# pranoyr/attention-models

Hardware: AMD Instinct MI355X
Metric: ViTVQGAN 256px train-step images/sec (higher is better)
Workload: dtype f32; 1 GPU; BASELINE.json configs[2]: ViTVQGAN dim=256 patch=8 img=256 depth=6+6 h=8 d=64 mlp=2048 (SwiGLU), codebook 8192x32; GAN train step (D phase + G phase, gradient penalty, per_loss_weight=0), Adam, clip 1.0; global_batch=32, batch_per_gpu=32, parallelism=dp1

## Files before the change

attention-models_amd/amk/dense.py:

```python
import ctypes

import torch

from . import lib as _lib
from .lib import EPI_BIAS, EPI_RESID, EPI_SWIGLU, EPI_SWIGLU_BWD, GEMM_NN, GEMM_NT, GEMM_TN, GemmDesc


def _p(t):
    return ctypes.c_void_p(t.data_ptr()) if t is not None else ctypes.c_void_p(0)


def _stream():
    return ctypes.c_void_p(torch.cuda.current_stream().cuda_stream)


def _mat(t, what):
    if t is None:
        return None
    if not t.is_cuda:
        raise RuntimeError("amk ops run only on MI355X (HIP) tensors; got a CPU tensor. There is no CPU fallback.")
    if t.dtype != torch.float32:
        raise RuntimeError(f"amk kernels compute in fp32; got {t.dtype} for {what}")
    if t.dim() != 2:
        raise RuntimeError(f"{what} must be a matrix, got shape {tuple(t.shape)}")
    if t.stride(1) != 1 or t.stride(0) % 4 or t.data_ptr() % 16:
        t = t.contiguous()
    return t


def _vec(t, n, what):
    if t is None:
        return None
    if not t.is_cuda or t.dtype != torch.float32:
        raise RuntimeError(f"{what}: an fp32 HIP tensor is required")
    t = t.contiguous()
    if t.numel() != n:
        raise RuntimeError(f"{what}: {t.numel()} elements, expected {n}")
    return t


def supported(*dims):
    return all(d > 0 and d % 4 == 0 for d in dims)


def _run(d, ws=None):
    L = _lib.load()
    rc = L.amk_gemm_f32(ctypes.byref(d), _p(ws), ws.numel() * 4 if ws is not None else 0, _stream())
    _lib.check(rc, "amk_gemm_f32")


def _set_ln(d, ln, M, K):
    if ln is None:
        return ()
    mean, rstd, gamma, beta = ln
    keep = (_vec(mean, M, "ln mean"), _vec(rstd, M, "ln rstd"), _vec(gamma, K, "ln gamma"), _vec(beta, K, "ln beta"))
    d.ln_mean, d.ln_rstd, d.ln_gamma, d.ln_beta = (_p(t) for t in keep)
    return keep


def row_stats(x2, eps=1e-5):
    x2 = _mat(x2, "x")
    M, D = x2.shape
    if x2.stride(0) != D:
        x2 = x2.contiguous()
    mean = torch.empty((M,), device=x2.device, dtype=torch.float32)
    rstd = torch.empty_like(mean)
    _lib.check(_lib.load().amk_row_stats(_p(x2), M, D, float(eps), _p(mean), _p(rstd), _stream()), "amk_row_stats")
    return mean, rstd


def gemm_nt(a, w, bias=None, *, w2=None, bias2=None, resid=None, ln=None, out=None):
    a, w, w2, resid = _mat(a, "a"), _mat(w, "w"), _mat(w2, "w2"), _mat(resid, "resid")
    M, K = a.shape
    N1 = w.shape[0]
    N2 = w2.shape[0] if w2 is not None else 0
    if w.shape[1] != K or (w2 is not None and w2.shape[1] != K):
        raise RuntimeError(f"gemm_nt: a {tuple(a.shape)} against w {tuple(w.shape)}")
    c = out if out is not None else torch.empty((M, N1), device=a.device, dtype=torch.float32)
    c2 = torch.empty((M, N2), device=a.device, dtype=torch.float32) if w2 is not None else None
    d = GemmDesc(op=GEMM_NT, epilogue=EPI_RESID if resid is not None else EPI_BIAS, m=M, n=N1 + N2, k=K,
                 split=N1 if w2 is not None else 0)
    bias, bias2 = _vec(bias, N1, "bias"), _vec(bias2, N2, "bias2")
    d.a, d.lda, d.w, d.ldw, d.c, d.ldc, d.bias = _p(a), a.stride(0), _p(w), w.stride(0), _p(c), c.stride(0), _p(bias)
    if w2 is not None:
        d.w2, d.ldw2, d.c2, d.ldc2, d.bias2 = _p(w2), w2.stride(0), _p(c2), c2.stride(0), _p(bias2)
    if resid is not None:
        if resid.shape != (M, N1):
            raise RuntimeError(f"gemm_nt: resid {tuple(resid.shape)} against output {(M, N1)}")
        d.resid, d.ldr = _p(resid), resid.stride(0)
    keep = _set_ln(d, ln, M, K)
    _run(d)
    return (c, c2) if w2 is not None else c


def gemm_nt_swiglu(a, w12, b12=None, *, ln=None, keep_ab=True):
    a, w12 = _mat(a, "a"), _mat(w12, "w12")
    M, K = a.shape
    H = w12.shape[0] // 2
    if w12.shape[1] != K or w12.shape[0] != 2 * H:
        raise RuntimeError(f"gemm_nt_swiglu: a {tuple(a.shape)} against w12 {tuple(w12.shape)}")
    gate = torch.empty((M, H), device=a.device, dtype=torch.float32)
    ab = torch.empty((M, 2 * H), device=a.device, dtype=torch.float32) if keep_ab else None
    d = GemmDesc(op=GEMM_NT, epilogue=EPI_SWIGLU, m=M, n=H, k=K)
    b12 = _vec(b12, 2 * H, "b12")
    d.a, d.lda, d.w, d.ldw, d.bias = _p(a), a.stride(0), _p(w12), w12.stride(0), _p(b12)
    d.gate, d.ldg = _p(gate), H
    d.c, d.ldc = _p(ab), 2 * H
    keep = _set_ln(d, ln, M, K)
    _run(d)
    return gate, ab


def gemm_nn(a, w, *, a2=None, w2=None, swiglu_ab=None):
    a, w, a2, w2, swiglu_ab = _mat(a, "a"), _mat(w, "w"), _mat(a2, "a2"), _mat(w2, "w2"), _mat(swiglu_ab, "ab")
    M, K1 = a.shape
    N = w.shape[1]
    K2 = a2.shape[1] if a2 is not None else 0
    if w.shape[0] != K1 or (a2 is not None and (w2 is None or w2.shape != (K2, N) or a2.shape[0] != M)):
        raise RuntimeError(f"gemm_nn: a {tuple(a.shape)} against w {tuple(w.shape)}")
    width = 2 * N if swiglu_ab is not None else N
    c = torch.empty((M, width), device=a.device, dtype=torch.float32)
    d = GemmDesc(op=GEMM_NN, epilogue=EPI_SWIGLU_BWD if swiglu_ab is not None else EPI_BIAS, m=M, n=N, k=K1 + K2,
                 split=K1 if a2 is not None else 0)
    d.a, d.lda, d.w, d.ldw, d.c, d.ldc = _p(a), a.stride(0), _p(w), w.stride(0), _p(c), width
    if a2 is not None:
        d.a2, d.lda2, d.w2, d.ldw2 = _p(a2), a2.stride(0), _p(w2), w2.stride(0)
    if swiglu_ab is not None:
        if swiglu_ab.shape != (M, 2 * N):
            raise RuntimeError(f"gemm_nn: (a | b) {tuple(swiglu_ab.shape)} against dGate {(M, N)}")
        d.ab, d.ldab = _p(swiglu_ab), swiglu_ab.stride(0)
    _run(d)
    return c


def _out(t, shape, what):
    if t is None:
        return None
    if (not t.is_cuda or t.dtype != torch.float32 or tuple(t.shape) != tuple(shape) or not t.is_contiguous()
            or t.data_ptr() % 16):
        raise RuntimeError(f"{what}: an fp32 contiguous 16-byte aligned HIP tensor of shape {tuple(shape)} is required")
    return t


def gemm_tn(y, x, *, y2=None, ln=None, want_bias=False, out=None, out2=None, bias_out=None):
    y, x, y2 = _mat(y, "y"), _mat(x, "x"), _mat(y2, "y2")
    M, N1 = y.shape
    K = x.shape[1]
    N2 = y2.shape[1] if y2 is not None else 0
    if x.shape[0] != M or (y2 is not None and y2.shape[0] != M):
        raise RuntimeError(f"gemm_tn: y {tuple(y.shape)} against x {tuple(x.shape)}")
    dw = _out(out, (N1, K), "gemm_tn out")
    if dw is None:
        dw = torch.empty((N1, K), device=y.device, dtype=torch.float32)
    dw2 = None
    if y2 is not None:
        dw2 = _out(out2, (N2, K), "gemm_tn out2")
        if dw2 is None:
            dw2 = torch.empty((N2, K), device=y.device, dtype=torch.float32)
    db = None
    if want_bias:
        db = _out(bias_out, (N1 + N2,), "gemm_tn bias_out")
        if db is None:
            db = torch.empty((N1 + N2,), device=y.device, dtype=torch.float32)
    d = GemmDesc(op=GEMM_TN, epilogue=EPI_BIAS, m=M, n=N1 + N2, k=K, split=N1 if y2 is not None else 0)
    d.a, d.lda, d.w, d.ldw, d.c, d.ldc, d.dbias = _p(y), y.stride(0), _p(x), x.stride(0), _p(dw), K, _p(db)
    if y2 is not None:
        d.a2, d.lda2, d.c2, d.ldc2 = _p(y2), y2.stride(0), _p(dw2), K
    keep = _set_ln(d, ln, M, K)
    L = _lib.load()
    nbytes = L.amk_gemm_f32_ws_bytes(ctypes.byref(d))
    ws = torch.empty((nbytes // 4,), device=y.device, dtype=torch.float32) if nbytes else None
    _run(d, ws)
    return dw, dw2, db


def _mat16(t, what):
    if not t.is_cuda:
        raise RuntimeError("amk ops run only on MI355X (HIP) tensors; got a CPU tensor. There is no CPU fallback.")
    if t.dtype != torch.bfloat16 or t.dim() != 2:
        raise RuntimeError(f"{what} must be a bf16 matrix, got {t.dtype} {tuple(t.shape)}")
    if t.stride(1) != 1 or t.stride(0) % 8 or t.data_ptr() % 16:
        t = t.contiguous()
    return t


def supported_bf16(N, K):
    return N > 0 and K > 0 and N % 8 == 0 and K % 8 == 0


def gemm_tn_bf16(y, x, want_bias=False, out=None, bias_out=None):
    y, x = _mat16(y, "y"), _mat16(x, "x")
    M, N = y.shape
    K = x.shape[1]
    if x.shape[0] != M:
        raise RuntimeError(f"gemm_tn_bf16: y has {M} rows, x {x.shape[0]}")
    if not supported_bf16(N, K):
        raise RuntimeError(f"gemm_tn_bf16: N and K must be multiples of 8, got {N}, {K}")
    L = _lib.load()
    dw = _out(out, (N, K), "gemm_tn_bf16 out")
    if dw is None:
        dw = torch.empty(N, K, device=y.device, dtype=torch.float32)
    db = None
    if want_bias:
        db = _out(bias_out, (N,), "gemm_tn_bf16 bias_out")
        if db is None:
            db = torch.empty(N, device=y.device, dtype=torch.float32)
    nbytes = L.amk_gemm_tn_bf16_ws_bytes(M, N, K)
    ws = torch.empty(nbytes // 4, device=y.device, dtype=torch.float32) if nbytes else None
    rc = L.amk_gemm_tn_bf16(_p(y), y.stride(0), _p(x), x.stride(0), _p(dw), K, _p(db), M, N, K, _p(ws), nbytes, _stream())
    _lib.check(rc, "amk_gemm_tn_bf16")
    return dw, db


def _bias32(bias, n):
    if bias is None:
        return None
    if bias.dtype != torch.float32 or not bias.is_cuda:
        raise RuntimeError("gemm bf16: the bias stays in fp32 (it is added to the fp32 accumulators)")
    bias = bias.contiguous()
    if bias.numel() != n or bias.data_ptr() % 16:
        raise RuntimeError(f"gemm bf16: bias of {bias.numel()} elements (16-byte aligned) expected {n}")
    return bias


def gemm_nt_bf16(a, w, bias=None):
    a, w = _mat16(a, "a"), _mat16(w, "w")
    (M, K), N = a.shape, w.shape[0]
    if w.shape[1] != K or not supported_bf16(N, K):
        raise RuntimeError(f"gemm_nt_bf16: a {tuple(a.shape)} x w {tuple(w.shape)}^T (multiples of 8 required)")
    bias = _bias32(bias, N)
    c = torch.empty(M, N, device=a.device, dtype=torch.bfloat16)
    if M:
        rc = _lib.load().amk_gemm_bf16(0, 0, _p(a), a.stride(0), _p(w), w.stride(0), _p(bias), _p(c), N, _p(None), 0, M, N, K, _stream())
        _lib.check(rc, "amk_gemm_bf16")
    return c


def gemm_nn_bf16(a, w):
    a, w = _mat16(a, "a"), _mat16(w, "w")
    (M, K), N = a.shape, w.shape[1]
    if w.shape[0] != K or not supported_bf16(N, K):
        raise RuntimeError(f"gemm_nn_bf16: a {tuple(a.shape)} x w {tuple(w.shape)} (multiples of 8 required)")
    c = torch.empty(M, N, device=a.device, dtype=torch.bfloat16)
    if M:
        rc = _lib.load().amk_gemm_bf16(1, 0, _p(a), a.stride(0), _p(w), w.stride(0), _p(None), _p(c), N, _p(None), 0, M, N, K, _stream())
        _lib.check(rc, "amk_gemm_bf16")
    return c


def gemm_nt_swiglu_bf16(a, w12, b12=None, keep_ab=True):
    a, w12 = _mat16(a, "a"), _mat16(w12, "w12")
    (M, K), N = a.shape, w12.shape[0]
    if w12.shape[1] != K or N % 16 or K % 8:
        raise RuntimeError(f"gemm_nt_swiglu_bf16: a {tuple(a.shape)} x w12 {tuple(w12.shape)}^T (2 H a multiple of 16, K of 8)")
    b12 = _bias32(b12, N)
    g = torch.empty(M, N // 2, device=a.device, dtype=torch.bfloat16)
    ab = torch.empty(M, N, device=a.device, dtype=torch.bfloat16) if keep_ab else None
    if M:
        rc = _lib.load().amk_gemm_bf16(0, 1, _p(a), a.stride(0), _p(w12), w12.stride(0), _p(b12), _p(ab), N, _p(g), N // 2, M, N, K, _stream())
        _lib.check(rc, "amk_gemm_bf16")
    return g, ab


def gemm_nn_swiglu_bwd_bf16(dy, w3, ab):
    dy, w3, ab = _mat16(dy, "dy"), _mat16(w3, "w3"), _mat16(ab, "ab")
    (M, K), H = dy.shape, w3.shape[1]
    if w3.shape[0] != K or ab.shape != (M, 2 * H) or not supported_bf16(H, K):
        raise RuntimeError(f"gemm_nn_swiglu_bwd_bf16: dy {tuple(dy.shape)}, w3 {tuple(w3.shape)}, ab {tuple(ab.shape)}")
    dab = torch.empty(M, 2 * H, device=dy.device, dtype=torch.bfloat16)
    if M:
        rc = _lib.load().amk_gemm_bf16_swiglu_bwd(_p(dy), dy.stride(0), _p(w3), w3.stride(0), _p(ab), ab.stride(0), _p(dab), 2 * H,
                                                  M, H, K, _stream())
        _lib.check(rc, "amk_gemm_bf16_swiglu_bwd")
    return dab
```

attention-models_amd/amk/lib.py:

```python
import ctypes
import os
import re

_HERE = os.path.dirname(os.path.abspath(__file__))
LIB_PATH = os.environ.get("AMK_LIB") or os.path.join(_HERE, "libamk.so")
HEADER_PATH = os.path.normpath(os.path.join(_HERE, "..", "..", "include", "amk.h"))

AMK_OK = 0

_c = ctypes
_P = _c.c_void_p
_I = _c.c_int
_L = _c.c_int64
_F = _c.c_float



class GemmDesc(_c.Structure):
    _fields_ = [("op", _c.c_int32), ("epilogue", _c.c_int32), ("m", _L),
                ("n", _c.c_int32), ("k", _c.c_int32), ("split", _c.c_int32), ("reserved", _c.c_int32),
                ("a", _P), ("a2", _P), ("w", _P), ("w2", _P), ("c", _P), ("c2", _P),
                ("lda", _L), ("lda2", _L), ("ldw", _L), ("ldw2", _L), ("ldc", _L), ("ldc2", _L),
                ("bias", _P), ("bias2", _P), ("resid", _P), ("ldr", _L),
                ("ln_mean", _P), ("ln_rstd", _P), ("ln_gamma", _P), ("ln_beta", _P),
                ("ab", _P), ("ldab", _L), ("gate", _P), ("ldg", _L), ("dbias", _P)]


GEMM_NT, GEMM_NN, GEMM_TN = 0, 1, 2
EPI_BIAS, EPI_RESID, EPI_SWIGLU, EPI_SWIGLU_BWD = 0, 1, 2, 3

SIGNATURES = {
    "amk_version": (_I, []),
    "amk_arch": (_c.c_char_p, []),
    "amk_last_error": (_c.c_char_p, []),
    "amk_attn_fwd": (_I, [_P] * 7 + [_I] * 5 + [_L] * 12 + [_F, _P]),
    "amk_attn_scores_bytes": (_L, [_I, _I, _I, _I]),
    "amk_attn_fwd_keep": (_I, [_P] * 8 + [_I] * 5 + [_L] * 12 + [_F, _P]),
    "amk_attn_fwd_x6_ws_bytes": (_L, [_I, _I, _I]),
    "amk_attn_fwd_x6": (_I, [_P] * 8 + [_I] * 5 + [_L] * 12 + [_F, _P]),
    "amk_attn_bwd_ws_floats": (_L, [_I, _I, _I, _I, _I]),
    "amk_attn_bwd": (_I, [_P] * 12 + [_I] * 5 + [_L] * 24 + [_F, _I, _P]),
    "amk_attn_bwd_kept": (_I, [_P] * 13 + [_I] * 5 + [_L] * 24 + [_F, _I, _P]),
    "amk_vq_num_partials": (_L, [_L]),
    "amk_vq_lookup_fwd": (_I, [_P, _P, _L, _I, _I, _I] + [_P] * 9 + [_P]),
    "amk_vq_lookup_bwd": (_I, [_P] * 7 + [_F, _L, _I, _I, _P, _P, _P]),
    "amk_vq_lookup_bwd_rows": (_I, [_P] * 7 + [_F, _L, _I, _I, _P, _P, _P]),
    "amk_vq_padded_codes": (_I, [_I, _I]),
    "amk_vq_gather": (_I, [_P, _P, _L, _I, _I, _P, _P, _P]),
    "amk_agent_num_chunks": (_I, [_I]),
    "amk_agent_ws_floats": (_L, [_I, _I, _I, _I, _I]),
    "amk_agent_num_chunks_dh": (_I, [_I, _I]),
    "amk_agent_ws_floats_dh": (_L, [_I, _I, _I, _I, _I, _I]),
    "amk_agent_attn_fwd": (_I, [_P] * 10 + [_I] * 5 + [_L] * 12 + [_F, _P]),
    "amk_agent_attn_bwd": (_I, [_P] * 14 + [_I] * 5 + [_L] * 21 + [_F, _P]),
    "amk_agent_conv_grad_reduce": (_I, [_P, _P, _L, _I, _P, _P, _P]),
    "amk_rowsum_num_partials": (_I, [_L]),
    "amk_add_layernorm_fwd": (_I, [_P, _P, _P, _P, _L, _I, _F, _P, _P, _P, _P, _P]),
    "amk_add_layernorm_bwd": (_I, [_P, _P, _P, _P, _P, _P, _L, _I, _P, _P, _P]),
    "amk_colsum": (_I, [_P, _L, _I, _P, _P]),
    "amk_swiglu_fwd": (_I, [_P, _L, _I, _P, _P]),
    "amk_swiglu_bwd": (_I, [_P, _P, _L, _I, _P, _P]),
    "amk_geglu_fwd": (_I, [_P, _L, _I, _P, _P]),
    "amk_geglu_bwd": (_I, [_P, _P, _L, _I, _P, _P]),
    "amk_opt_num_partials": (_I, []),
    "amk_sumsq_partials": (_I, [_P, _L, _P, _P]),
    "amk_adam_flat_step": (_I, [_P] * 4 + [_L, _P, _P, _P, _I] + [_F] * 6 + [_I, _P, _P]),
    "amk_adam_flat_step_shadow": (_I, [_P] * 4 + [_L, _P, _P, _P, _I] + [_F] * 6 + [_I, _P, _P, _P]),
    "amk_gemm_x6_planes_bytes": (_L, [_I, _I]),
    "amk_gemm_x6_split": (_I, [_P, _L, _I, _I, _P, _P]),
    "amk_gemm_x6_nt": (_I, [_P, _L, _P, _P, _P, _L, _I, _I, _I, _P]),
    "amk_gemm_f32_ws_bytes": (_L, [_c.POINTER(GemmDesc)]),
    "amk_gemm_f32": (_I, [_c.POINTER(GemmDesc), _P, _L, _P]),
    "amk_row_stats": (_I, [_P, _L, _I, _F, _P, _P, _P]),
    "amk_attn_bf16_fwd": (_I, [_P] * 7 + [_I] * 5 + [_L] * 12 + [_F, _P]),
    "amk_attn_bf16_bwd_ws_floats": (_L, [_I, _I, _I, _I]),
    "amk_attn_bf16_bwd": (_I, [_P] * 12 + [_I] * 5 + [_L] * 24 + [_F, _P]),
    "amk_swiglu_bf16_fwd": (_I, [_P, _L, _I, _P, _P]),
    "amk_swiglu_bf16_bwd": (_I, [_P, _P, _L, _I, _P, _P]),
    "amk_add_layernorm_mixed_fwd": (_I, [_P, _I, _P, _P, _P, _L, _I, _F, _P, _P, _P, _P, _P]),
    "amk_add_layernorm_mixed_bwd": (_I, [_P, _I, _P, _P, _P, _P, _P, _L, _I, _P, _P, _P, _P]),
    "amk_gemm_bf16": (_I, [_I, _I, _P, _L, _P, _L, _P, _P, _L, _P, _L, _L, _I, _I, _P]),
    "amk_gemm_bf16_swiglu_bwd": (_I, [_P, _L, _P, _L, _P, _L, _P, _L, _L, _I, _I, _P]),
    "amk_gemm_tn_bf16_ws_bytes": (_L, [_L, _I, _I]),
    "amk_gemm_tn_bf16": (_I, [_P, _L, _P, _L, _P, _L, _P, _L, _I, _I, _P, _L, _P]),
    "amk_sample_step": (_I, [_P, _P, _F, _P, _c.c_uint64, _c.c_uint64, _F, _L, _I, _I, _P, _F, _P, _P, _P]),
    "amk_moe_route_ws_ints": (_L, [_L, _I, _I]),
    "amk_moe_route": (_I, [_P, _L, _I, _I] + [_P] * 8),
    "amk_grouped_gemm_nt": (_I, [_P, _L, _I, _P, _P, _P, _P, _L, _I, _I, _I, _P, _P]),
    "amk_grouped_gemm_nn": (_I, [_P, _L, _I, _P, _P, _P, _P, _L, _I, _I, _I, _P, _P]),
    "amk_grouped_gemm_nt_acc": (_I, [_P, _L, _I, _P, _P, _P, _P, _L, _I, _I, _I, _P, _I, _P]),
    "amk_grouped_gemm_nn_acc": (_I, [_P, _L, _I, _P, _P, _P, _P, _L, _I, _I, _I, _P, _I, _P]),
    "amk_grouped_gemm_wgrad": (_I, [_P, _L, _I, _P, _L, _I, _P, _P, _P, _L, _I, _I, _I, _P, _P, _P]),
    "amk_moe_combine": (_I, [_P, _P, _P, _L, _I, _I, _I, _P, _P]),
    "amk_moe_expert_sums": (_I, [_P, _L, _I, _P, _P, _L, _I, _I, _I, _P, _P]),
    "amk_moe_topk": (_I, [_P, _L, _I, _I, _P, _P, _P]),
    "amk_moe_route_distinct": (_I, [_P, _L, _I, _I, _P, _P, _P, _P]),
    "amk_moe_combine_rows": (_I, [_P, _P, _P, _L, _I, _I, _I, _I, _I, _P, _P]),
    "amk_moe_gate_grad_rows": (_I, [_P, _P, _P, _P, _L, _I, _I, _I, _I, _I, _P, _P]),
    "amk_moe_gate_grad": (_I, [_P, _P, _P, _P, _L, _I, _I, _I, _I, _P, _P]),
    "amk_bnact_ws_floats": (_L, [_I, _I, _L]),
    "amk_bnact_fwd": (_I, [_P, _P, _P, _I, _I, _L, _F, _F, _F] + [_P] * 7),
    "amk_bnact_bwd": (_I, [_P] * 6 + [_I, _I, _L, _F] + [_P] * 6),
    "amk_bnact_bwd_bwd": (_I, [_P] * 10 + [_I, _I, _L, _F] + [_P] * 5),
}

_lib = None


def declared_symbols(header_path=HEADER_PATH):
    text = open(header_path).read()
    text = re.sub(r"/\*.*?\*/", "", text, flags=re.S)
    return sorted(set(re.findall(r"\b(amk_[a-z0-9_]+)\s*\(", text)))


def load():
    global _lib
    if _lib is not None:
        return _lib
    if not os.path.exists(LIB_PATH):
        raise RuntimeError(
            f"{LIB_PATH} is missing: build it with `python -c 'import __graft_entry__ as g; g.build()'` "
            "(hipcc --offload-arch=gfx950). amk has no CPU or eager fallback."
        )
    lib = ctypes.CDLL(LIB_PATH)
    for name, (res, args) in SIGNATURES.items():
        fn = getattr(lib, name)
        fn.restype = res
        fn.argtypes = args
    arch = lib.amk_arch().decode()
    if arch != "gfx950":
        raise RuntimeError(f"libamk.so was built for {arch}, expected gfx950")
    _lib = lib
    return lib


def check(rc, what):
    if rc != AMK_OK:
        msg = load().amk_last_error().decode()
        raise RuntimeError(f"{what} failed with code {rc}: {msg}")
```

attention-models_amd/amk/ops.py:

```python
import ctypes
import os
import weakref

import torch
from torch.autograd.function import once_differentiable

from . import lib as _lib

_NULL = ctypes.c_void_p(0)


def _ptr(t):
    return ctypes.c_void_p(t.data_ptr()) if t is not None else _NULL


def _stream():
    return ctypes.c_void_p(torch.cuda.current_stream().cuda_stream)


KERNEL_EVENTS = None


class _timed:

# ... 614 lines not shown
    U, E = logits2.shape
    ids = torch.empty((U, k), device=logits2.device, dtype=torch.int64)
    gate = torch.empty((U, k), device=logits2.device, dtype=torch.float32)
    _lib.check(_lib.load().amk_moe_topk(_ptr(logits2.contiguous()), U, E, k, _ptr(ids), _ptr(gate), _stream()), "amk_moe_topk")
    return ids, gate


def _route_distinct(ids, G, fan, E):
    dev = ids.device
    mask = torch.empty((G,), device=dev, dtype=torch.int64)
    offsets, perm = _i32(E + 1, dev), _i32(G * min(fan, E), dev)
    _lib.check(_lib.load().amk_moe_route_distinct(_ptr(ids), G, fan, E, _ptr(mask), _ptr(offsets), _ptr(perm), _stream()),
               "amk_moe_route_distinct")
    return offsets, perm


def distinct_experts_ok(dim, d, fan, E, *weights):
    return E <= 64 and _moe_dense_z(dim, d, fan, E) and dim % 4 == 0 and all(w.is_cuda for w in weights)


class _SharedRowExperts(torch.autograd.Function):

    @staticmethod
    @_amp_fwd
    def forward(ctx, x2, logits2, W, k, H):
        _require_device(x2, logits2, W)
        x2, W = x2.contiguous(), W.contiguous()
        U, E = logits2.shape
        N, Kd = W.shape[1], W.shape[2]
        G, fan = U // H, H * k
        if x2.shape != (G, Kd) or U % H:
            raise RuntimeError(f"shared-row experts: shapes disagree: x {tuple(x2.shape)} U {U} H {H} W {tuple(W.shape)}")
        L = _lib.load()
        with _timed(f"moe_topk U{U} E{E} k{k} + distinct lists"):
            ids, gate = _topk(logits2.detach(), k)
            offsets, perm = _route_distinct(ids, G, fan, E)
        V = torch.empty((G * E, N), device=x2.device, dtype=torch.float32)
        with _timed(f"grouped_nt P{U * k} N{N} K{Kd} (distinct rows)"):
            _lib.check(L.amk_grouped_gemm_nt(_ptr(x2), Kd, E, _ptr(W), _NULL, _ptr(offsets), _ptr(perm), G * E, E, N, Kd, _ptr(V),
                                             _stream()), "amk_grouped_gemm_nt")
        out = torch.empty((U, N), device=x2.device, dtype=torch.float32)
        _lib.check(L.amk_moe_combine_rows(_ptr(V), _ptr(ids), _ptr(gate), U, 1, k, N, fan, E, _ptr(out), _stream()),
                   "amk_moe_combine_rows")
        ctx.save_for_backward(x2, W, V, ids, gate, offsets, perm)
        ctx.cfg = (k, H)
        ctx.mark_non_differentiable(ids)
        ctx.set_materialize_grads(False)
        return out, ids

    @staticmethod
    @once_differentiable
    @_amp_bwd
    def backward(ctx, d_out, _d_ids):
        if d_out is None:
            return (None,) * 5
        x2, W, V, ids, gate, offsets, perm = ctx.saved_tensors
        k, H = ctx.cfg
        E, N, Kd = W.shape
        G, fan = x2.shape[0], H * k
        U = G * H
        d_out = d_out.contiguous()
        L = _lib.load()
        dlogits = torch.empty((U, E), device=x2.device, dtype=torch.float32)
        _lib.check(L.amk_moe_gate_grad_rows(_ptr(d_out), _ptr(V), _ptr(ids), _ptr(gate), U * k, k, E, N, k, fan, _ptr(dlogits),
                                            _stream()), "amk_moe_gate_grad_rows")
        Z = _expert_sums(d_out, k, ids, _ptr(gate), G, fan, E, N)
        dx = None
        if ctx.needs_input_grad[0]:
            with _timed(f"dense_z_gemm M{G} N{Kd} K{E * N}"):
                dx = Z @ W.view(E * N, Kd)
        dW = torch.empty_like(W)
        with _timed(f"grouped_wgrad P{U * k} N{N} K{Kd} (distinct rows)"):
            _lib.check(L.amk_grouped_gemm_wgrad(_ptr(Z), N, 1, _ptr(x2), Kd, E, _NULL, _ptr(offsets), _ptr(perm), G * E, E, N, Kd,
                                                _ptr(dW), _NULL, _stream()), "amk_grouped_gemm_wgrad")
        return dx, dlogits, dW, None, None


class _SummedExperts(torch.autograd.Function):

    @staticmethod
    @_amp_fwd
    def forward(ctx, a2, logits2, W, k, H):
        _require_device(a2, logits2, W)
        a2, W = a2.contiguous(), W.contiguous()
        U, E = logits2.shape
        N, Kd = W.shape[1], W.shape[2]
        G, fan = U // H, H * k
        if a2.shape != (U, Kd) or U % H:
            raise RuntimeError(f"summed experts: shapes disagree: a {tuple(a2.shape)} U {U} H {H} W {tuple(W.shape)}")
        with _timed(f"moe_topk U{U} E{E} k{k}"):
            ids, _gate = _topk(logits2.detach(), k)
        Z = _expert_sums(a2, k, ids, _NULL, G, fan, E, Kd)
        with _timed(f"dense_z_gemm M{G} N{N} K{E * Kd}"):
            out = Z @ W.permute(0, 2, 1).reshape(E * Kd, N)
        ctx.save_for_backward(W, Z, ids)
        ctx.cfg = (k, H)
        ctx.mark_non_differentiable(ids)
        ctx.set_materialize_grads(False)
        return out, ids

    @staticmethod
    @once_differentiable
    @_amp_bwd
    def backward(ctx, d_out, _d_ids):
        if d_out is None:
            return (None,) * 5
        W, Z, ids = ctx.saved_tensors
        k, H = ctx.cfg
        E, N, Kd = W.shape
        G, fan = Z.shape[0], H * k
        U = G * H
        d_out = d_out.contiguous()
        L = _lib.load()
        offsets, perm = _route_distinct(ids, G, fan, E)
        da = None
        if ctx.needs_input_grad[0]:
            D = torch.empty((G * E, Kd), device=W.device, dtype=torch.float32)
            with _timed(f"grouped_nn P{U * k} N{N} K{Kd} (distinct rows)"):
                _lib.check(L.amk_grouped_gemm_nn(_ptr(d_out), N, E, _ptr(W), _NULL, _ptr(offsets), _ptr(perm), G * E, E, N, Kd, _ptr(D),
                                                 _stream()), "amk_grouped_gemm_nn")
            da = torch.empty((U, Kd), device=W.device, dtype=torch.float32)
            _lib.check(L.amk_moe_combine_rows(_ptr(D), _ptr(ids), _NULL, U, 1, k, Kd, fan, E, _ptr(da), _stream()),
                       "amk_moe_combine_rows")
        dW = torch.empty_like(W)
        with _timed(f"grouped_wgrad P{U * k} N{N} K{Kd} (distinct rows)"):
            _lib.check(L.amk_grouped_gemm_wgrad(_ptr(d_out), N, E, _ptr(Z), Kd, 1, _NULL, _ptr(offsets), _ptr(perm), G * E, E, N, Kd,
                                                _ptr(dW), _NULL, _stream()), "amk_grouped_gemm_wgrad")
        return da, None, dW, None, None


def shared_row_experts(x2, logits2, W, k, H):
    return _SharedRowExperts.apply(x2, logits2, W, k, H)


def summed_experts(a2, logits2, W, k, H):
    return _SummedExperts.apply(a2, logits2, W, k, H)


class _AgentAttn(torch.autograd.Function):

    @staticmethod
    @_amp_fwd
    def forward(ctx, qkv2, conv_w, conv_b, H, D, P, scale):
        _require_device(qkv2, conv_w, conv_b)
        B, T, _ = qkv2.shape
        qkv2 = qkv2.contiguous()
        qkv = qkv2.view(B, T, 3, H, D)
        q, k, v = (qkv[:, :, j].permute(0, 2, 1, 3) for j in range(3))
        dev = qkv2.device
        o = _new_bthd(B, H, T, D, qkv2)
        agents = torch.empty((B, H, P, D), device=dev, dtype=torch.float32)
        vagent = torch.empty_like(agents)
        stats1 = torch.empty((B, H, P, 2), device=dev, dtype=torch.float32)
        cw, cb = conv_w.contiguous(), conv_b.contiguous()
        L = _lib.load()
        ws = torch.empty((max(L.amk_agent_ws_floats_dh(B, H, T, P, D, 0), 1),), device=dev, dtype=torch.float32)
        rc = L.amk_agent_attn_fwd(_ptr(q), _ptr(k), _ptr(v), _ptr(cw), _ptr(cb), _ptr(o), _ptr(agents), _ptr(vagent),
                                  _ptr(stats1), _ptr(ws), B, H, T, D, P, *_strides4(q), *_strides4(k), *_strides4(v), *_strides4(o),
                                  float(scale), _stream())
        _lib.check(rc, "amk_agent_attn_fwd")
        ctx.save_for_backward(qkv2, cw, agents, vagent, stats1)
        ctx.cfg = (H, D, P, scale)
        return o.permute(0, 2, 1, 3).reshape(B, T, H * D)

    @staticmethod
    @once_differentiable
    @_amp_bwd
    def backward(ctx, d_o2):
        qkv2, cw, agents, vagent, stats1 = ctx.saved_tensors
        H, D, P, scale = ctx.cfg
        B, T, _ = qkv2.shape
        dev = qkv2.device
        qkv = qkv2.view(B, T, 3, H, D)
        q, k, v = (qkv[:, :, j].permute(0, 2, 1, 3) for j in range(3))
        d_o = d_o2.contiguous().view(B, T, H, D).permute(0, 2, 1, 3)
        dqkv2 = torch.empty_like(qkv2)
        dqkv = dqkv2.view(B, T, 3, H, D)
        dq, dk, dv = (dqkv[:, :, j].permute(0, 2, 1, 3) for j in range(3))
        L = _lib.load()
        cells = B * H * L.amk_agent_num_chunks_dh(T, D)
        ws = torch.empty((max(L.amk_agent_ws_floats_dh(B, H, T, P, D, 1), 1),), device=dev, dtype=torch.float32)
        dw_part = torch.empty((cells, 9, D), device=dev, dtype=torch.float32)
        db_part = torch.empty((cells, D), device=dev, dtype=torch.float32)
        rc = L.amk_agent_attn_bwd(_ptr(q), _ptr(k), _ptr(v), _ptr(cw), _ptr(d_o), _ptr(agents), _ptr(vagent), _ptr(stats1),
                                  _ptr(dq), _ptr(dk), _ptr(dv), _ptr(ws), _ptr(dw_part), _ptr(db_part),
                                  B, H, T, D, P, *_strides4(q), *_strides4(k), *_strides4(v), *_strides4(d_o),
                                  *_strides4(dq), *_strides4(dk), *_strides4(dv), float(scale), _stream())
        _lib.check(rc, "amk_agent_attn_bwd")
        dconv_w = torch.empty((D, 1, 3, 3), device=dev, dtype=torch.float32)
        dconv_b = torch.empty((D,), device=dev, dtype=torch.float32)
        _lib.check(L.amk_agent_conv_grad_reduce(_ptr(dw_part), _ptr(db_part), cells, D, _ptr(dconv_w), _ptr(dconv_b), _stream()),
                   "amk_agent_conv_grad_reduce")
        return dqkv2, dconv_w, dconv_b, None, None, None, None


def agent_attention(qkv2, conv_w, conv_b, num_heads, dim_head, pool, scale):
    return _AgentAttn.apply(qkv2, conv_w, conv_b, num_heads, dim_head, pool, scale)


class _SwiGLU(torch.autograd.Function):
    FWD, BWD = "amk_swiglu_fwd", "amk_swiglu_bwd"

    @classmethod
    def forward(cls, ctx, ab):
        _require_device(ab)
        H = ab.shape[-1] // 2
        ab2 = ab.contiguous().view(-1, 2 * H)
        M = ab2.shape[0]
        out = torch.empty((M, H), device=ab.device, dtype=torch.float32)
        L = _lib.load()
        _lib.check(getattr(L, cls.FWD)(_ptr(ab2), M, H, _ptr(out), _stream()), cls.FWD)
        ctx.save_for_backward(ab2)
        ctx.shape = ab.shape
        return out.view(*ab.shape[:-1], H)

    @classmethod
    def backward(cls, ctx, d_out):
        (ab2,) = ctx.saved_tensors
        M, H2 = ab2.shape
        d_out = d_out.contiguous().view(M, H2 // 2)
        d_ab = torch.empty_like(ab2)
        L = _lib.load()
        _lib.check(getattr(L, cls.BWD)(_ptr(ab2), _ptr(d_out), M, H2 // 2, _ptr(d_ab), _stream()), cls.BWD)
        return d_ab.view(ctx.shape)


class _GEGLU(_SwiGLU):
    FWD, BWD = "amk_geglu_fwd", "amk_geglu_bwd"


def _f32_outside_autocast(fn, x):
    if torch.is_autocast_enabled():
        with torch.autocast("cuda", enabled=False):
            return fn(x.float())
    return fn(x)


class _SwiGLUBF16(torch.autograd.Function):

    @staticmethod
    def forward(ctx, ab):
        H = ab.shape[-1] // 2
        ab2 = ab.contiguous().view(-1, 2 * H)
        M = ab2.shape[0]
        out = torch.empty((M, H), device=ab.device, dtype=torch.bfloat16)
        _lib.check(_lib.load().amk_swiglu_bf16_fwd(_ptr(ab2), M, H, _ptr(out), _stream()), "amk_swiglu_bf16_fwd")
        ctx.save_for_backward(ab2)
        ctx.shape = ab.shape
        return out.view(*ab.shape[:-1], H)

    @staticmethod
    @once_differentiable
    def backward(ctx, d_out):
        (ab2,) = ctx.saved_tensors
        M, H2 = ab2.shape
        d_out = d_out.to(torch.bfloat16).contiguous().view(M, H2 // 2)
        d_ab = torch.empty_like(ab2)
        _lib.check(_lib.load().amk_swiglu_bf16_bwd(_ptr(ab2), _ptr(d_out), M, H2 // 2, _ptr(d_ab), _stream()), "amk_swiglu_bf16_bwd")
        return d_ab.view(ctx.shape)


MIXED_ELEMENTWISE = os.environ.get("AMK_MIXED_ELEMENTWISE", "1") == "1"


def swiglu(ab):
    if MIXED_ELEMENTWISE and ab.dtype == torch.bfloat16 and ab.is_cuda and ab.shape[-1] % 8 == 0:
        with torch.autocast("cuda", enabled=False):
            return _SwiGLUBF16.apply(ab)
    return _f32_outside_autocast(_SwiGLU.apply, ab)


def geglu(ab):
    return _f32_outside_autocast(_GEGLU.apply, ab)


def _ln_supported(D):
    return 0 < D <= 4096 and D % 4 == 0


def _ln_param_grads(part, params):
    weight, bias = params if params is not None else (None, None)
    (wr, wv), (br, bv) = _claim_late(weight), _claim_late(bias)
    if wv is None and bv is None:
        dgb = part.sum(0)
        return dgb[0], dgb[1]
    dw = db = None
    if wv is not None:
        torch.sum(part[:, 0], dim=0, out=wv)
        wr.wrote(weight)
    else:
        dw = part[:, 0].sum(0)
    if bv is not None:
        torch.sum(part[:, 1], dim=0, out=bv)
        br.wrote(bias)
    else:
        db = part[:, 1].sum(0)
    return dw, db


def _claim_late(p):
    return _claim(p)


def _ln_backward(dy, h, dh_in, weight, mean, rstd, params=None):
    M, D = h.shape
    L = _lib.load()
    dh = torch.empty_like(h)
    part = torch.empty((L.amk_rowsum_num_partials(M), 2, D), device=h.device, dtype=torch.float32)
    _lib.check(L.amk_add_layernorm_bwd(_ptr(dy), _ptr(h), _ptr(dh_in), _ptr(weight), _ptr(mean), _ptr(rstd),
                                       M, D, _ptr(dh), _ptr(part), _stream()), "amk_add_layernorm_bwd")
    dw, db = _ln_param_grads(part, params)
    return dh, dw, db


class _LayerNorm(torch.autograd.Function):
    @staticmethod
    @_amp_fwd
    def forward(ctx, x, weight, bias, eps):
        _require_device(x, weight, bias)
        D = x.shape[-1]
        x2 = x.contiguous().view(-1, D)
        M = x2.shape[0]
        y = torch.empty_like(x2)
        mean = torch.empty((M,), device=x.device, dtype=torch.float32)
        rstd = torch.empty_like(mean)
        w, b = weight.contiguous(), bias.contiguous()
        L = _lib.load()
        _lib.check(L.amk_add_layernorm_fwd(_ptr(x2), _NULL, _ptr(w), _ptr(b), M, D, float(eps), _NULL, _ptr(y),
                                           _ptr(mean), _ptr(rstd), _stream()), "amk_add_layernorm_fwd")
        ctx.save_for_backward(x2, w, mean, rstd)
        ctx.shape = x.shape
        ctx.params = (weight, bias)
        return y.view(x.shape)

    @staticmethod
    @once_differentiable
    @_amp_bwd
    def backward(ctx, dy):
        x2, w, mean, rstd = ctx.saved_tensors
        dx, dw, db = _ln_backward(dy.contiguous().view(x2.shape), x2, None, w, mean, rstd, ctx.params)
        return dx.view(ctx.shape), dw, db, None


class _AddLayerNorm(torch.autograd.Function):

    @staticmethod
    @_amp_fwd
    def forward(ctx, x, res, weight, bias, eps):
        _require_device(x, res, weight, bias)
        D = x.shape[-1]
        x2 = x.contiguous().view(-1, D)
        r2 = res.contiguous().view(-1, D)
        M = x2.shape[0]
        h = torch.empty_like(x2)
        y = torch.empty_like(x2)
        mean = torch.empty((M,), device=x.device, dtype=torch.float32)
        rstd = torch.empty_like(mean)
        w, b = weight.contiguous(), bias.contiguous()
        L = _lib.load()
        _lib.check(L.amk_add_layernorm_fwd(_ptr(x2), _ptr(r2), _ptr(w), _ptr(b), M, D, float(eps), _ptr(h), _ptr(y),
                                           _ptr(mean), _ptr(rstd), _stream()), "amk_add_layernorm_fwd")
        ctx.save_for_backward(h, w, mean, rstd)
        ctx.shape = x.shape
        ctx.params = (weight, bias)
        ctx.set_materialize_grads(False)
        return h.view(x.shape), y.view(x.shape)

    @staticmethod
    @once_differentiable
    @_amp_bwd
    def backward(ctx, dh_in, dy):
        h, w, mean, rstd = ctx.saved_tensors
        if dy is None:
            if dh_in is None:
                return None, None, None, None, None
            return dh_in, dh_in, None, None, None
        dh2 = dh_in.contiguous().view(h.shape) if dh_in is not None else None
        dh, dw, db = _ln_backward(dy.contiguous().view(h.shape), h, dh2, w, mean, rstd, ctx.params)
        dh = dh.view(ctx.shape)
        return dh, dh, dw, db, None


class _AddLayerNormMixed(torch.autograd.Function):

    @staticmethod
    def forward(ctx, x, res, weight, bias, eps):
        _require_device(res, weight, bias)
        D = x.shape[-1]
        x2 = x.contiguous().view(-1, D)
        M = x2.shape[0]
        xb = x2.dtype == torch.bfloat16
        if not xb and x2.dtype != torch.float32:
            raise RuntimeError(f"mixed LayerNorm takes f32 or bf16 inputs, got {x2.dtype}")
        r2 = res.contiguous().view(-1, D) if res is not None else None
        need_h = r2 is not None or xb
        h = torch.empty((M, D), device=x.device, dtype=torch.float32) if need_h else None
        y = torch.empty((M, D), device=x.device, dtype=torch.bfloat16)
        mean = torch.empty((M,), device=x.device, dtype=torch.float32)
        rstd = torch.empty_like(mean)
        w, b = weight.contiguous(), bias.contiguous()
        _lib.check(_lib.load().amk_add_layernorm_mixed_fwd(_ptr(x2), 1 if xb else 0, _ptr(r2), _ptr(w), _ptr(b), M, D, float(eps),
                                                          _ptr(h), _ptr(y), _ptr(mean), _ptr(rstd), _stream()),
                   "amk_add_layernorm_mixed_fwd")
        hs = h if need_h else x2
        ctx.save_for_backward(hs, w, mean, rstd)
        ctx.cfg = (x.shape, xb, res is not None)
        ctx.params = (weight, bias)
        ctx.set_materialize_grads(False)
        return hs.view(x.shape), y.view(x.shape)

    @staticmethod
    @once_differentiable
    def backward(ctx, dh_in, dy):
        h, w, mean, rstd = ctx.saved_tensors
        shape, xb, has_res = ctx.cfg
        M, D = h.shape
        if dy is None:
            if dh_in is None:
                return None, None, None, None, None
            dx = dh_in.to(torch.bfloat16) if xb else dh_in
            return dx, (dh_in if has_res else None), None, None, None
        dyb = dy.dtype == torch.bfloat16
        dy2 = (dy if dyb else dy.float()).contiguous().view(M, D)
        dh2 = dh_in.float().contiguous().view(M, D) if dh_in is not None else None
        L = _lib.load()
        dh = torch.empty((M, D), device=h.device, dtype=torch.float32)
        dh16 = torch.empty((M, D), device=h.device, dtype=torch.bfloat16) if xb else None
        part = torch.empty((L.amk_rowsum_num_partials(M), 2, D), device=h.device, dtype=torch.float32)
        _lib.check(L.amk_add_layernorm_mixed_bwd(_ptr(dy2), 1 if dyb else 0, _ptr(h), _ptr(dh2), _ptr(w), _ptr(mean), _ptr(rstd),
                                                 M, D, _ptr(dh), _ptr(dh16), _ptr(part), _stream()), "amk_add_layernorm_mixed_bwd")
        dw, db = _ln_param_grads(part, ctx.params)
        dhv = dh.view(shape)
        dx = dh16.view(shape) if xb else dhv
        return dx, (dhv if has_res else None), dw, db, None


def _mixed_ln():
    return (MIXED_ELEMENTWISE and torch.is_autocast_enabled() and torch.get_autocast_dtype("cuda") == torch.bfloat16)


def layer_norm(x, weight, bias, eps=1e-5, branch=False):
    if not _ln_supported(x.shape[-1]) or x.numel() == 0 or not x.is_cuda:
        return torch.nn.functional.layer_norm(x, (x.shape[-1],), weight, bias, eps)
    if branch and _mixed_ln():
        with torch.autocast("cuda", enabled=False):
            return _AddLayerNormMixed.apply(x, None, weight, bias, eps)[1]
    return _LayerNorm.apply(x, weight, bias, eps)


def add_layer_norm(x, res, weight, bias, eps=1e-5, branch=False):
    if not _ln_supported(x.shape[-1]) or x.numel() == 0 or not x.is_cuda:
        h = x + res
        return h, torch.nn.functional.layer_norm(h, (h.shape[-1],), weight, bias, eps)
    if branch and _mixed_ln():
        with torch.autocast("cuda", enabled=False):
            return _AddLayerNormMixed.apply(x, res.float(), weight, bias, eps)
    return _AddLayerNorm.apply(x, res, weight, bias, eps)


def colsum(x2):
    M, N = x2.shape
    if N % 4 != 0 or N > 1024:
        return x2.sum(0)
    L = _lib.load()
    part = torch.empty((L.amk_rowsum_num_partials(M), N), device=x2.device, dtype=torch.float32)
    _lib.check(L.amk_colsum(_ptr(x2), M, N, _ptr(part), _stream()), "amk_colsum")
    return part.sum(0)


class _BiasLinear(torch.autograd.Function):

    @staticmethod
    def forward(ctx, x, weight, bias):
        _require_device(x, weight, bias)
        ctx.save_for_backward(x, weight)
        return torch.nn.functional.linear(x, weight, bias)

    @staticmethod
    @once_differentiable
    def backward(ctx, dy):
        x, weight = ctx.saved_tensors
        dy2 = dy.contiguous().view(-1, dy.shape[-1])
        dx = dy2.mm(weight).view(x.shape) if ctx.needs_input_grad[0] else None
        dw = dy2.t().mm(x.reshape(-1, x.shape[-1])) if ctx.needs_input_grad[1] else None
        db = colsum(dy2) if ctx.needs_input_grad[2] else None
        return dx, dw, db


GEMM_MODE = os.environ.get("AMK_GEMM", "f32")


def gemm_x6_nt(a2, b2, bias=None):
    _require_device(a2, b2, bias)
    if a2.stride(1) != 1:
        a2 = a2.contiguous()
    if b2.stride(1) != 1:
        b2 = b2.contiguous()
    M, K = a2.shape
    N = b2.shape[0]
    L = _lib.load()
    planes = torch.empty((L.amk_gemm_x6_planes_bytes(N, K),), device=a2.device, dtype=torch.uint8)
    c = torch.empty((M, N), device=a2.device, dtype=torch.float32)
    with _timed(f"gemm_x6_nt M{M} N{N} K{K}"):
        _lib.check(L.amk_gemm_x6_split(_ptr(b2), b2.stride(0), N, K, _ptr(planes), _stream()), "amk_gemm_x6_split")
        rc = L.amk_gemm_x6_nt(_ptr(a2), a2.stride(0), _ptr(planes), _ptr(bias), _ptr(c), N, M, N, K, _stream())
    _lib.check(rc, "amk_gemm_x6_nt")
    return c


def _x6_ok(x, weight):
    K = weight.shape[1]
    if K % 4 or x.numel() == 0 or x.data_ptr() % 16 or weight.data_ptr() % 16:
        return False
    if x.stride(-1) != 1 or (x.dim() >= 2 and x.stride(-2) % 4):
        return False
    return x.numel() * 4 < 0x7ffffff0 and weight.numel() * 8 < 0x7ffffff0


class _LinearX6(torch.autograd.Function):

    @staticmethod
    def forward(ctx, x, weight, bias):
        _require_device(x, weight, bias)
        x2 = x.reshape(-1, x.shape[-1])
        ctx.save_for_backward(x2, weight)
        ctx.x_shape = x.shape
        ctx.has_bias = bias is not None
        return gemm_x6_nt(x2, weight, bias).view(*x.shape[:-1], weight.shape[0])

    @staticmethod
    @once_differentiable
    def backward(ctx, dy):
        x2, weight = ctx.saved_tensors
        dy2 = dy.contiguous().view(-1, dy.shape[-1])
        dx = dw = db = None
        if ctx.needs_input_grad[0]:
            N = weight.shape[0]
            if N % 4 == 0:
                dx = gemm_x6_nt(dy2, weight.t().contiguous()).view(ctx.x_shape)
            else:
                dx = dy2.mm(weight).view(ctx.x_shape)
        if ctx.needs_input_grad[1]:
            dw = dy2.t().mm(x2)
        if ctx.has_bias and ctx.needs_input_grad[2]:
            db = colsum(dy2)
        return dx, dw, db


DENSE_MODE = os.environ.get("AMK_DENSE", "auto")


DENSE_AUTO_MAX_K = int(os.environ.get("AMK_DENSE_MAX_K", "512"))


def _dense_ok(x, *weights):
    if DENSE_MODE == "lib" or torch.is_autocast_enabled() or not x.is_cuda or x.dtype != torch.float32 or x.numel() == 0:
        return False
    if x.shape[-1] % 4 or x.shape[-1] < 128:
        return False
    if DENSE_MODE == "auto" and x.shape[-1] > DENSE_AUTO_MAX_K:
        return False
    return all(w.dtype == torch.float32 and w.shape[0] % 4 == 0 and w.shape[0] >= 128 and w.is_contiguous() for w in weights)


def _nn_plain(dy2, weight):
    from . import dense

    if DENSE_MODE == "amk":
        return dense.gemm_nn(dy2, weight)
    return dy2.mm(weight)


def _claim(p):
    ref = getattr(p, "_amk_reducer", None) if p is not None else None
    red = ref() if ref is not None else None
    if red is None:
        return None, None
    view = red.claim(p)
    return (red, view) if view is not None else (None, None)


class _DenseLinear(torch.autograd.Function):

    @staticmethod
    def forward(ctx, x, weight, bias):
        from . import dense

        x2 = x.reshape(-1, x.shape[-1])
        ctx.save_for_backward(x2, weight)
        ctx.x_shape = x.shape
        ctx.has_bias = bias is not None
        ctx.params = (weight, bias)
        if DENSE_MODE == "auto" and weight.shape[0] < 512:
            return torch.nn.functional.linear(x, weight, bias)
        return dense.gemm_nt(x2, weight, bias).view(*x.shape[:-1], weight.shape[0])

    @staticmethod
    @once_differentiable
    def backward(ctx, dy):
        from . import dense

        x2, weight = ctx.saved_tensors
        dy2 = dy.reshape(-1, dy.shape[-1])
        dx = dw = db = None
        if ctx.needs_input_grad[0]:
            dx = _nn_plain(dy2, weight).view(ctx.x_shape)
        if ctx.needs_input_grad[1] or (ctx.has_bias and ctx.needs_input_grad[2]):
            want_b = ctx.has_bias and ctx.needs_input_grad[2]
            (wr, wv), (br, bv) = _claim(ctx.params[0]), (_claim(ctx.params[1]) if want_b else (None, None))
            dw, _, db = dense.gemm_tn(dy2, x2, want_bias=want_b, out=wv, bias_out=bv)
            if wv is not None:
                wr.wrote(ctx.params[0])
                dw = None
            if bv is not None:
# ... 297 lines not shown
```

attention-models_amd/csrc/amk_common.h:

```cpp
#pragma once
#include <hip/hip_runtime.h>
#include <stdint.h>
#include <stdarg.h>
#include <stdio.h>
#include "../../include/amk.h"

typedef float f32x16 __attribute__((ext_vector_type(16)));
typedef float f32x4 __attribute__((ext_vector_type(4)));

#define AMK_WAVE 64
#define AMK_LOG2E 1.4426950408889634f
#define AMK_LN2 0.6931471805599453f

void amk_set_error(const char* fmt, ...);

#define AMK_CHECK_ARG(cond, ...)        \
  do {                                  \
    if (!(cond)) {                      \
      amk_set_error(__VA_ARGS__);       \
      return AMK_EINVAL;                \
    }                                   \
  } while (0)

#define AMK_CHECK_SUPPORTED(cond, ...)  \
  do {                                  \
    if (!(cond)) {                      \
      amk_set_error(__VA_ARGS__);       \
      return AMK_EUNSUPPORTED;          \
    }                                   \
  } while (0)

#define AMK_CHECK_LAUNCH(what)                                              \
  do {                                                                      \
    hipError_t e_ = hipGetLastError();                                      \
    if (e_ != hipSuccess) {                                                 \
      amk_set_error("%s: %s", what, hipGetErrorString(e_));                 \
      return AMK_ELAUNCH;                                                   \
    }                                                                       \
  } while (0)

__device__ __forceinline__ f32x16 mfma32(float a, float b, f32x16 c) {
  return __builtin_amdgcn_mfma_f32_32x32x2f32(a, b, c, 0, 0, 0);
}

__device__ __forceinline__ constexpr int acc_row(int r, int hf) {
  return (r & 3) + 8 * (r >> 2) + 4 * hf;
}

__device__ __forceinline__ int xcd_remap(int bid, int nwg) {
  const int q = nwg >> 3, r = nwg & 7, xcd = bid & 7;
  const int base = (xcd < r) ? xcd * (q + 1) : r * (q + 1) + (xcd - r) * q;
  return base + (bid >> 3);
}

__device__ __forceinline__ float wave_xor32_max(float x) {
  return fmaxf(x, __shfl_xor(x, 32, 64));
}
```

attention-models_amd/csrc/gemm_f32.hip:

```cpp
#include "amk_common.h"
#include <stdlib.h>
#include <string.h>
#include <type_traits>

#ifndef AMK_DENSE_DEFAULT_BK
#define AMK_DENSE_DEFAULT_BK 32
#endif

namespace amk_dense {

constexpr int LSC = 132;
constexpr unsigned ROW_PAST = 0x40000000u;
constexpr unsigned K_PAST = 0x80000000u;

template <int BK>
struct Geo {
  static constexpr int LSR = BK + 4;
  static constexpr int BREG = 128 * LSR;
  static constexpr int STAGE = 2 * BREG;
  static constexpr int NG = BK / 8;
  static constexpr int NP = BK / 8;
  static constexpr int TPR = BK / 4;
  static constexpr int RPP = 256 / TPR;
  static_assert(BK == 16 || BK == 32, "BK");
  static_assert(BK * LSC <= BREG, "the C image must fit the operand region");
};

__device__ __forceinline__ float4 ld4(const float* p) { return *reinterpret_cast<const float4*>(p); }
__device__ __forceinline__ void st4(float* p, float4 v) { *reinterpret_cast<float4*>(p) = v; }
__device__ __forceinline__ f32x16 zero16() {
  f32x16 z;
#pragma unroll
  for (int i = 0; i < 16; ++i) z[i] = 0.f;
  return z;
}
__device__ __forceinline__ float4 bload4(__amdgpu_buffer_rsrc_t r, int off) {
  return __builtin_bit_cast(float4, __builtin_amdgcn_raw_buffer_load_b128(r, off, 0, 0));
}
__device__ __forceinline__ float bload1(__amdgpu_buffer_rsrc_t r, int off) {
  return __builtin_bit_cast(float, __builtin_amdgcn_raw_buffer_load_b32(r, off, 0, 0));
}
__device__ __forceinline__ void bstore1(float v, __amdgpu_buffer_rsrc_t r, int off) {
  __builtin_amdgcn_raw_buffer_store_b32(__builtin_bit_cast(unsigned, v), r, off, 0, 0);
}
__device__ __forceinline__ __amdgpu_buffer_rsrc_t mkrsrc(const void* base, int64_t bytes) {
  return __builtin_amdgcn_make_buffer_rsrc((void*)base, 0, (int)(bytes < 0 ? 0 : (bytes > 0x3FFFFFFF ? 0x3FFFFFFF : bytes)), 0x00020000);
}
__device__ __forceinline__ float sigmoidf_(float x) { return 1.f / (1.f + expf(-x)); }

__device__ __forceinline__ void lds_barrier() {
  __builtin_amdgcn_fence(__ATOMIC_RELEASE, "workgroup", "local");
  __builtin_amdgcn_s_barrier();
  __builtin_amdgcn_fence(__ATOMIC_ACQUIRE, "workgroup", "local");
}

enum { EPI_BIAS = 0, EPI_RESID = 1, EPI_SWIGLU = 2, EPI_SWIGLU_BWD = 3 };

struct Params {
  const float *a, *a2, *w, *w2, *bias, *bias2, *resid;
  float *c, *c2;
  const float *ln_mean, *ln_rstd, *ln_gamma, *ln_beta;
  const float* ab;
  float* gate;
  float* dbias;
  float* ws;
  int64_t lda, lda2, ldw, ldw2, ldc, ldc2, ldr, ldab, ldg;
  int64_t M;
  int N, K, split, H;
  int ntn, total;
  int nchunk, steps_per_chunk;
  int stagger_mode, stagger_sleeps;
};

__device__ __forceinline__ void stagger(const Params& p, int slots) {
  if (p.stagger_mode == 0 || (int)blockIdx.x >= slots) return;
  const int k = blockIdx.x >> 3;
  const int late = p.stagger_mode == 1 ? (k >> 5) & 1 : (p.stagger_mode == 2 ? k & 1 : ((k >> 5) ^ k) & 1);
  if (late) {
    for (int i = 0; i < p.stagger_sleeps; ++i) __builtin_amdgcn_s_sleep(127);
  }
}

__device__ __forceinline__ void lane_offsets(unsigned (&vo)[4], int hf, int64_t ld, unsigned colbytes) {
#pragma unroll
  for (int e = 0; e < 4; ++e) vo[e] = (unsigned)((4 * hf + e) * ld * 4) + colbytes;
}
__device__ __forceinline__ __amdgpu_buffer_rsrc_t group_rsrc(const float* base, int64_t ld, int rows, int rg0, int col0, int width) {
  int n = rows - rg0;
  n = n > 8 ? 8 : n;
  return mkrsrc(base + (int64_t)rg0 * ld + col0, n > 0 ? ((int64_t)(n - 1) * ld + width) * 4 : 0);
}

#ifndef AMK_DENSE_EDGE_PRIO
#define AMK_DENSE_EDGE_PRIO 3
#endif
#ifndef AMK_DENSE_MOVE_PRIO
#define AMK_DENSE_MOVE_PRIO 0
#endif
template <int BK, bool ACT, bool BCT, class Mover>
__device__ __forceinline__ void step_loop(f32x16 (&acc)[2][2], float* smem, int nk, int a_rd, int a_blk, int b_rd,
                                          int b_blk, Mover& mv) {
  using G = Geo<BK>;
  for (int kt = 0; kt < nk; ++kt) {
    const float* cur = smem + (kt & 1) * G::STAGE;
    float* nxt = smem + ((kt + 1) & 1) * G::STAGE;
    float a[2][4], b[2][4];
    auto frag = [&](int s4, float (&fa)[2][4], float (&fb)[2][4]) {
#pragma unroll
      for (int i = 0; i < 2; ++i) {
        if constexpr (!ACT) {
          const float4 v = ld4(cur + a_rd + i * a_blk + 4 * s4);
          fa[i][0] = v.x; fa[i][1] = v.y; fa[i][2] = v.z; fa[i][3] = v.w;
        } else {
#pragma unroll
          for (int x = 0; x < 4; ++x) fa[i][x] = cur[a_rd + i * a_blk + (4 * s4 + x) * LSC];
        }
        if constexpr (!BCT) {
          const float4 v = ld4(cur + G::BREG + b_rd + i * b_blk + 4 * s4);
          fb[i][0] = v.x; fb[i][1] = v.y; fb[i][2] = v.z; fb[i][3] = v.w;
        } else {
#pragma unroll
          for (int x = 0; x < 4; ++x) fb[i][x] = cur[G::BREG + b_rd + i * b_blk + (4 * s4 + x) * LSC];
        }
      }
    };
#ifndef AMK_ABLATE
#define AMK_ABLATE 0
#endif
    if (!(AMK_ABLATE & 4) || kt == 0) frag(0, a, b);
#pragma unroll
    for (int s4 = 0; s4 < G::NG; ++s4) {
      float an[2][4], bn[2][4];
      if (s4 + 1 < G::NG) {
        if (!(AMK_ABLATE & 4)) frag(s4 + 1, an, bn);
        else {
#pragma unroll
          for (int i = 0; i < 2; ++i)
#pragma unroll
            for (int x = 0; x < 4; ++x) { an[i][x] = a[i][x]; bn[i][x] = b[i][x]; }
        }
      }
      if (AMK_DENSE_MOVE_PRIO) __builtin_amdgcn_s_setprio(AMK_DENSE_MOVE_PRIO);
      if (!(AMK_ABLATE & 1)) {
        mv(2 * s4, nxt, kt);
        mv(2 * s4 + 1, nxt, kt);
      }
      if (AMK_DENSE_MOVE_PRIO) __builtin_amdgcn_s_setprio(0);
      __builtin_amdgcn_sched_barrier(0);
#pragma unroll
      for (int x = 0; x < 4; ++x) {
#pragma unroll
        for (int i = 0; i < 2; ++i) {
#pragma unroll
          for (int j = 0; j < 2; ++j) acc[i][j] = mfma32(a[i][x], b[j][x], acc[i][j]);
        }
      }
      __builtin_amdgcn_sched_barrier(0);
      if (s4 + 1 < G::NG) {
#pragma unroll
        for (int i = 0; i < 2; ++i) {
#pragma unroll
          for (int x = 0; x < 4; ++x) { a[i][x] = an[i][x]; b[i][x] = bn[i][x]; }
        }
      }
    }
    if (!(AMK_ABLATE & 2)) __syncthreads();
  }
}

#define AMK_DENSE_BOUNDS(BK) __launch_bounds__(256, (BK) == 16 ? 3 : 2)

template <int BK, int EPI, bool LNA>
__global__ AMK_DENSE_BOUNDS(BK) void gemm_nt_kernel(Params p) {
  using G = Geo<BK>;
  constexpr int NP = G::NP, LSR = G::LSR;
  __shared__ __attribute__((aligned(16))) float smem[2 * G::STAGE];
  const int tid = threadIdx.x, lane = tid & 63, wave = __builtin_amdgcn_readfirstlane(tid >> 6), ln = lane & 31, hf = lane >> 5;
  const int wm = wave >> 1, wn = wave & 1;
  stagger(p, (BK == 16 ? 3 : 2) * 256);
  __builtin_amdgcn_s_setprio(AMK_DENSE_EDGE_PRIO);
#ifdef AMK_DENSE_STAMPS
#define AMK_STAMP(i) do { if (tid == 0 && p.ws) reinterpret_cast<unsigned long long*>(p.ws)[(size_t)blockIdx.x * 8 + (i)] = __builtin_amdgcn_s_memrealtime(); } while (0)
  AMK_STAMP(0);
  if (tid == 0 && p.ws) {
    reinterpret_cast<unsigned long long*>(p.ws)[(size_t)blockIdx.x * 8 + 6] = __builtin_amdgcn_s_getreg((31 << 11) | (0 << 6) | 4);
    reinterpret_cast<unsigned long long*>(p.ws)[(size_t)blockIdx.x * 8 + 7] = __builtin_amdgcn_s_getreg((31 << 11) | (0 << 6) | 20);
  }
#else
#define AMK_STAMP(i)
#endif
  const int u = xcd_remap(blockIdx.x, p.total);
  const int mt = u / p.ntn, nt = u - mt * p.ntn;
  const int64_t m0 = (int64_t)mt * 128;
  const int rows = (int)(p.M - m0 < 128 ? p.M - m0 : 128);
  constexpr bool SW = EPI == EPI_SWIGLU;
  int n0 = SW ? nt * 64 : nt * 128;
  const bool seg = !SW && p.split > 0 && n0 >= p.split;
  const float* Wb = seg ? p.w2 : p.w;
  const float* bias = seg ? p.bias2 : p.bias;
  float* Cb = seg ? p.c2 : p.c;
  const int64_t ldw = seg ? p.ldw2 : p.ldw, ldc = seg ? p.ldc2 : p.ldc;
  const int ncols = SW ? p.H : (p.split > 0 ? (seg ? p.N - p.split : p.split) : p.N);
  if (seg) n0 -= p.split;
  const int wrows = SW ? 2 * p.H : ncols;

  const int sr = tid / G::TPR, sc = (tid % G::TPR) * 4;
  const __amdgpu_buffer_rsrc_t a_rsrc = mkrsrc(p.a + m0 * p.lda, ((int64_t)(rows - 1) * p.lda + p.K) * 4);
  const __amdgpu_buffer_rsrc_t w_rsrc = mkrsrc(Wb, ((int64_t)(wrows - 1) * ldw + p.K) * 4);
  const __amdgpu_buffer_rsrc_t g_rsrc = mkrsrc(LNA ? p.ln_gamma : p.a, LNA ? (int64_t)p.K * 4 : 0);
  const __amdgpu_buffer_rsrc_t be_rsrc = mkrsrc(LNA ? p.ln_beta : p.a, LNA ? (int64_t)p.K * 4 : 0);
  unsigned goff[2 * NP];
#pragma unroll
  for (int j = 0; j < NP; ++j) goff[j] = (unsigned)(((int64_t)(sr + G::RPP * j) * p.lda + sc) * 4);
#pragma unroll
  for (int j = 0; j < NP; ++j) {
    const int rr = sr + G::RPP * j;
    int wr;
    bool ok;
    if (SW) { const int jj = n0 + (rr & 63); ok = jj < p.H; wr = (rr < 64 ? 0 : p.H) + jj; }
    else { wr = n0 + rr; ok = wr < ncols; }
    goff[NP + j] = ok ? (unsigned)(((int64_t)wr * ldw + sc) * 4) : ROW_PAST;
  }
  float rs[NP], mu[NP];
  if (LNA) {
    const __amdgpu_buffer_rsrc_t m_rsrc = mkrsrc(p.ln_mean + m0, (int64_t)rows * 4);
    const __amdgpu_buffer_rsrc_t r_rsrc = mkrsrc(p.ln_rstd + m0, (int64_t)rows * 4);
#pragma unroll
    for (int j = 0; j < NP; ++j) { mu[j] = bload1(m_rsrc, (sr + G::RPP * j) * 4); rs[j] = bload1(r_rsrc, (sr + G::RPP * j) * 4); }
  }
  float4 stg[2 * NP], gam, bet;
  const int nk = (p.K + BK - 1) / BK;
  auto kadd = [&](int kt) {
    const int k0 = (kt < nk ? kt : nk - 1) * BK;
    return (k0 + sc < p.K) ? (unsigned)(k0 * 4) : K_PAST;
  };
  auto gload = [&](int i, unsigned ka) {
    if (i < NP) stg[i] = bload4(a_rsrc, (int)(goff[i] + ka));
    else stg[i] = bload4(w_rsrc, (int)(goff[i] + ka));
  };
  auto lstore = [&](int i, float* stage) {
    float4 v = stg[i];
    if (LNA && i < NP) {
      v.x = fmaf((v.x - mu[i]) * rs[i], gam.x, bet.x); v.y = fmaf((v.y - mu[i]) * rs[i], gam.y, bet.y);
      v.z = fmaf((v.z - mu[i]) * rs[i], gam.z, bet.z); v.w = fmaf((v.w - mu[i]) * rs[i], gam.w, bet.w);
    }
    st4(&stage[(i < NP ? 0 : G::BREG) + (sr + G::RPP * (i % NP)) * LSR + sc], v);
  };
  auto gbload = [&](unsigned ka) {
    if (LNA) { gam = bload4(g_rsrc, (int)(ka + sc * 4)); bet = bload4(be_rsrc, (int)(ka + sc * 4)); }
  };
  f32x16 acc[2][2];
#pragma unroll
  for (int i = 0; i < 2; ++i)
#pragma unroll
    for (int j = 0; j < 2; ++j) acc[i][j] = zero16();

  unsigned ka = kadd(0);
  gbload(ka);
#pragma unroll
  for (int i = 0; i < 2 * NP; ++i) gload(i, ka);
#pragma unroll
  for (int i = 0; i < 2 * NP; ++i) lstore(i, smem);
  ka = kadd(1);
  gbload(ka);
#pragma unroll
  for (int i = 0; i < 2 * NP; ++i) gload(i, ka);
  __syncthreads();
  AMK_STAMP(1);

  unsigned ka2 = 0;
  auto mv = [&](int i, float* nxt, int kt) {
    if (i == 0) ka2 = kadd(kt + 2);
    lstore(i, nxt);
    if (i == NP - 1) gbload(ka2);
    gload(i, ka2);
  };
  const int a_rd = (64 * wm + ln) * LSR + (BK / 2) * hf;
  const int b_rd = ((SW ? 32 : 64) * wn + ln) * LSR + (BK / 2) * hf;
  __builtin_amdgcn_s_setprio(0);
  step_loop<BK, false, false>(acc, smem, nk, a_rd, 32 * LSR, b_rd, (SW ? 64 : 32) * LSR, mv);
  __builtin_amdgcn_s_setprio(AMK_DENSE_EDGE_PRIO);
  AMK_STAMP(2);

  if constexpr (SW) {
    const int j = n0 + 32 * wn + ln;
    const bool ok = j < p.H;
    const float ba = (bias && ok) ? bias[j] : 0.f, bb = (bias && ok) ? bias[p.H + j] : 0.f;
    const unsigned cg = ok ? (unsigned)j * 4u : K_PAST;
    unsigned vg[4], vc[4];
    lane_offsets(vg, hf, p.ldg, cg);
    lane_offsets(vc, hf, ldc, cg);
    const float* gbase = p.gate + m0 * p.ldg;
    const float* abase = Cb ? Cb + m0 * ldc : p.gate;
#pragma unroll
    for (int i = 0; i < 2; ++i) {
#pragma unroll
      for (int q = 0; q < 4; ++q) {
        const int rg0 = 64 * wm + 32 * i + 8 * q;
        const __amdgpu_buffer_rsrc_t gr = group_rsrc(gbase, p.ldg, rows, rg0, 0, p.H);
        const __amdgpu_buffer_rsrc_t ar = group_rsrc(abase, ldc, Cb ? rows : 0, rg0, 0, p.H);
        const __amdgpu_buffer_rsrc_t br = group_rsrc(abase, ldc, Cb ? rows : 0, rg0, p.H, p.H);
#pragma unroll
        for (int e = 0; e < 4; ++e) {
          const float av = acc[i][0][4 * q + e] + ba, bv = acc[i][1][4 * q + e] + bb;
          bstore1(av * sigmoidf_(av) * bv, gr, (int)vg[e]);
          if (Cb) { bstore1(av, ar, (int)vc[e]); bstore1(bv, br, (int)vc[e]); }
        }
      }
    }
    return;
  }
  const float* cbase = Cb + m0 * ldc;
  const float* rbase = EPI == EPI_RESID ? p.resid + m0 * p.ldr : p.a;
#pragma unroll
  for (int j = 0; j < 2; ++j) {
    const int n = n0 + 64 * wn + 32 * j + ln;
    const bool ok = n < ncols;
    const float bv = (bias && ok) ? bias[n] : 0.f;
    const unsigned cn = ok ? (unsigned)n * 4u : K_PAST;
    unsigned vo[4], vr[4];
    lane_offsets(vo, hf, ldc, cn);
    if (EPI == EPI_RESID) lane_offsets(vr, hf, p.ldr, cn);
#pragma unroll
    for (int i = 0; i < 2; ++i) {
      float res[16];
      if (EPI == EPI_RESID) {
#pragma unroll
        for (int q = 0; q < 4; ++q) {
          const __amdgpu_buffer_rsrc_t rr = group_rsrc(rbase, p.ldr, rows, 64 * wm + 32 * i + 8 * q, 0, ncols);
#pragma unroll
          for (int e = 0; e < 4; ++e) res[4 * q + e] = bload1(rr, (int)vr[e]);
        }
      }
#pragma unroll
      for (int q = 0; q < 4; ++q) {
        const __amdgpu_buffer_rsrc_t cr = group_rsrc(cbase, ldc, rows, 64 * wm + 32 * i + 8 * q, 0, ncols);
#pragma unroll
        for (int e = 0; e < 4; ++e) {
          float v = acc[i][j][4 * q + e] + bv;
          if (EPI == EPI_RESID) v += res[4 * q + e];
          bstore1(v, cr, (int)vo[e]);
        }
      }
    }
  }
  AMK_STAMP(3);
}

template <int EPI, bool LNA>
struct NtWalk {
  static constexpr int BK = 32;
  using G = Geo<32>;
  static constexpr int LSR = G::LSR;
  static constexpr bool SW = EPI == EPI_SWIGLU;
  const Params& p;
  int tid, sr, sc, ln, hf, wm, wn, nk;
  __amdgpu_buffer_rsrc_t a_rsrc, w_rsrc, g_rsrc, be_rsrc, m_rsrc, r_rsrc;
  unsigned goff[8], ka;
  float4 stg[8], gam, bet;
  float mu[4], rs[4];
  f32x16 accp[2][2];
  const float *cbase_d, *rbase_d, *gbase_d;
  int64_t ldc_d;
  int rows_d, ncols_d;
  bool keep_ab_d;
  unsigned vo[4], vr[4], vg[4], d1;
  float bias_d[2];
  float res[2][4];
// ... 96 lines not shown
      cbase_d = Cb + m0 * ldc_d;
      if (EPI == EPI_RESID) {
        lane_offsets(vr, hf, p.ldr, cn);
        rbase_d = p.resid + m0 * p.ldr;
        res_load(0, 0);
        res_load(0, 1);
      }
    }
  }
  __device__ __forceinline__ void res_load(int d, int q) {
    const int i = d & 1, j = d >> 1;
    const __amdgpu_buffer_rsrc_t rr = group_rsrc(rbase_d, p.ldr, rows_d, 64 * wm + 32 * i + 8 * q, 0, ncols_d);
#pragma unroll
    for (int e = 0; e < 4; ++e) res[q & 1][e] = bload1(rr, (int)(vr[e] + (j ? d1 : 0u)));
  }
  __device__ __forceinline__ void drain(int d, int g) {
    if constexpr (SW) {
      const int i = d & 1, q = 2 * (d >> 1) + (g >> 1);
      const int rg0 = 64 * wm + 32 * i + 8 * q;
      const __amdgpu_buffer_rsrc_t gr = group_rsrc(gbase_d, p.ldg, rows_d, rg0, 0, p.H);
      const __amdgpu_buffer_rsrc_t ar = group_rsrc(cbase_d, ldc_d, keep_ab_d ? rows_d : 0, rg0, 0, p.H);
      const __amdgpu_buffer_rsrc_t br = group_rsrc(cbase_d, ldc_d, keep_ab_d ? rows_d : 0, rg0, p.H, p.H);
#pragma unroll
      for (int e2 = 0; e2 < 2; ++e2) {
        const int e = 2 * (g & 1) + e2;
        const float av = accp[i][0][4 * q + e] + bias_d[0], bv = accp[i][1][4 * q + e] + bias_d[1];
        bstore1(av * sigmoidf_(av) * bv, gr, (int)vg[e]);
        bstore1(av, ar, (int)vo[e]);
        bstore1(bv, br, (int)vo[e]);
      }
    } else {
      const int i = d & 1, j = d >> 1, q = g;
      const __amdgpu_buffer_rsrc_t cr = group_rsrc(cbase_d, ldc_d, rows_d, 64 * wm + 32 * i + 8 * q, 0, ncols_d);
#pragma unroll
      for (int e = 0; e < 4; ++e) {
        float v = accp[i][j][4 * q + e] + bias_d[j];
        if (EPI == EPI_RESID) v += res[q & 1][e];
        bstore1(v, cr, (int)(vo[e] + (j ? d1 : 0u)));
      }
      if (EPI == EPI_RESID) {
        const int nxt = 4 * d + g + 2;
        if (nxt < 16) res_load(nxt >> 2, nxt & 3);
      }
    }
  }
};

template <int EPI, bool LNA>
__global__ __launch_bounds__(256, 2) void gemm_nt_dkernel(Params p) {
  using W = NtWalk<EPI, LNA>;
  using G = Geo<32>;
  constexpr int LSR = G::LSR;
  constexpr bool SW = EPI == EPI_SWIGLU;
  __shared__ __attribute__((aligned(16))) float smem[2 * G::STAGE];
  W U(p);
  const int Gd = gridDim.x;
  int cu = blockIdx.x;
  if (cu >= p.total) return;
  int lu = cu, lk = 0;
  U.load_unit(lu);
  auto advance = [&]() {
    if (++lk == U.nk) {
      lk = 0;
      lu = lu + Gd < p.total ? lu + Gd : lu;
      U.load_unit(lu);
    }
  };
  const int a_rd = (64 * U.wm + U.ln) * LSR + 16 * U.hf;
  const int b_rd = ((SW ? 32 : 64) * U.wn + U.ln) * LSR + 16 * U.hf;
  constexpr int a_blk = 32 * LSR, b_blk = (SW ? 64 : 32) * LSR;
  f32x16 acc[2][2];
#pragma unroll
  for (int i = 0; i < 2; ++i)
#pragma unroll
    for (int j = 0; j < 2; ++j) acc[i][j] = zero16();
#pragma unroll
  for (int i = 0; i < 8; ++i) U.gload(i, lk);
  advance();
#pragma unroll
  for (int i = 0; i < 8; ++i) U.lstore(i, smem);
#pragma unroll
  for (int i = 0; i < 8; ++i) U.gload(i, lk);
  advance();
  lds_barrier();
  int s = 0;
  auto frag = [&](const float* st, int s4, float (&fa)[2][4], float (&fb)[2][4]) {
#pragma unroll
    for (int i = 0; i < 2; ++i) {
      const float4 v = ld4(st + a_rd + i * a_blk + 4 * s4);
      fa[i][0] = v.x; fa[i][1] = v.y; fa[i][2] = v.z; fa[i][3] = v.w;
      const float4 w = ld4(st + G::BREG + b_rd + i * b_blk + 4 * s4);
      fb[i][0] = w.x; fb[i][1] = w.y; fb[i][2] = w.z; fb[i][3] = w.w;
    }
  };
#ifndef AMK_WALK_BARRIER_AT
#define AMK_WALK_BARRIER_AT 2
#endif
  float a[2][4], b[2][4];
  frag(smem, 0, a, b);
  auto step = [&](auto dtag) {
    constexpr int D = decltype(dtag)::value;
    constexpr int BAT = AMK_WALK_BARRIER_AT;
    const float* cur = smem + (s & 1) * G::STAGE;
    float* nxt = smem + ((s + 1) & 1) * G::STAGE;
    auto mv = [&](int i) { U.lstore(i, nxt); U.gload(i, lk); };
#pragma unroll
    for (int g = 0; g < 4; ++g) {
      float an[2][4], bn[2][4];
      if (g + 1 < 4) frag(cur, g + 1, an, bn);
      if (BAT == 3) { mv(2 * g); mv(2 * g + 1); }
      else if (g == 0) { mv(0); mv(1); mv(2); }
      else if (g == 1) { mv(3); mv(4); mv(5); }
      else if (g == 2) { mv(6); mv(7); }
      if (g == BAT || (BAT == 3 && g == 3)) { if (g == (BAT == 3 ? 3 : 2)) advance(); }
      if (D >= 0) U.drain(D, g);
      if (BAT == 2 && g == 3) frag(nxt, 0, an, bn);
      __builtin_amdgcn_sched_barrier(0);
#pragma unroll
      for (int x = 0; x < 4; ++x) {
#pragma unroll
        for (int i = 0; i < 2; ++i) {
#pragma unroll
          for (int j = 0; j < 2; ++j) acc[i][j] = mfma32(a[i][x], b[j][x], (D == 0 && g == 0 && x == 0) ? zero16() : acc[i][j]);
        }
      }
      __builtin_amdgcn_sched_barrier(0);
      if (BAT == 2 && g == 2) lds_barrier();
      if (g + 1 < 4 || BAT == 2) {
#pragma unroll
        for (int i = 0; i < 2; ++i)
#pragma unroll
          for (int x = 0; x < 4; ++x) { a[i][x] = an[i][x]; b[i][x] = bn[i][x]; }
      }
    }
    if (BAT == 3) { lds_barrier(); frag(nxt, 0, a, b); }
    ++s;
  };
  for (;;) {
    step(std::integral_constant<int, 0>{});
    step(std::integral_constant<int, 1>{});
    step(std::integral_constant<int, 2>{});
    step(std::integral_constant<int, 3>{});
    for (int kt = 4; kt < U.nk; ++kt) step(std::integral_constant<int, -1>{});
    U.retire(acc, cu);
    cu += Gd;
    if (cu >= p.total) break;
  }
#pragma unroll
  for (int d = 0; d < 4; ++d)
#pragma unroll
    for (int g = 0; g < 4; ++g) U.drain(d, g);
}

template <int BK, int EPI>
__global__ AMK_DENSE_BOUNDS(BK) void gemm_nn_kernel(Params p) {
  using G = Geo<BK>;
  constexpr int NP = G::NP, LSR = G::LSR;
  __shared__ __attribute__((aligned(16))) float smem[2 * G::STAGE];
  const int tid = threadIdx.x, lane = tid & 63, wave = __builtin_amdgcn_readfirstlane(tid >> 6), ln = lane & 31, hf = lane >> 5;
  const int wm = wave >> 1, wn = wave & 1;
  stagger(p, (BK == 16 ? 3 : 2) * 256);
  __builtin_amdgcn_s_setprio(AMK_DENSE_EDGE_PRIO);
  const int u = xcd_remap(blockIdx.x, p.total);
  const int mt = u / p.ntn, nt = u - mt * p.ntn;
  const int64_t m0 = (int64_t)mt * 128;
  const int rows = (int)(p.M - m0 < 128 ? p.M - m0 : 128);
  const int n0 = nt * 128;
  const int K0 = p.split > 0 ? p.split : p.K, K1 = p.K - K0;
  const int nk0 = (K0 + BK - 1) / BK, nk1 = (K1 + BK - 1) / BK, nk = nk0 + nk1;

  const int sr = tid / G::TPR, sc = (tid % G::TPR) * 4;
  const int cr = tid >> 5, cc = (tid & 31) * 4;
  const bool col_ok = n0 + cc < p.N;
  unsigned aoff0[NP], aoff1[NP], woff0[NP], woff1[NP];
#pragma unroll
  for (int j = 0; j < NP; ++j) {
    aoff0[j] = (unsigned)(((int64_t)(sr + G::RPP * j) * p.lda + sc) * 4);
    aoff1[j] = (unsigned)(((int64_t)(sr + G::RPP * j) * p.lda2 + sc) * 4);
    woff0[j] = col_ok ? (unsigned)(((int64_t)(cr + 8 * j) * p.ldw + n0 + cc) * 4) : ROW_PAST;
    woff1[j] = col_ok ? (unsigned)(((int64_t)(cr + 8 * j) * p.ldw2 + n0 + cc) * 4) : ROW_PAST;
  }
  float4 stg[2 * NP];
  auto seg_of = [&](int kt, int& s, int& k0) {
    const int t = kt < nk ? kt : nk - 1;
    s = t >= nk0;
    k0 = (s ? t - nk0 : t) * BK;
  };
  auto gload_tile_piece = [&](int i, int s, int k0) {
    const float* ab_ = s ? p.a2 : p.a;
    const int64_t lda = s ? p.lda2 : p.lda;
    const float* wb_ = s ? p.w2 : p.w;
    const int64_t ldw = s ? p.ldw2 : p.ldw;
    const int Ks = s ? K1 : K0;
    if (i < NP) {
      const __amdgpu_buffer_rsrc_t ar = mkrsrc(ab_ + m0 * lda, ((int64_t)(rows - 1) * lda + Ks) * 4);
      const unsigned off = (k0 + sc < Ks) ? (s ? aoff1[i] : aoff0[i]) + (unsigned)(k0 * 4) : K_PAST;
      stg[i] = bload4(ar, (int)off);
    } else {
      const __amdgpu_buffer_rsrc_t wr = mkrsrc(wb_, ((int64_t)(Ks - 1) * ldw + p.N) * 4);
      stg[i] = bload4(wr, (int)((s ? woff1[i - NP] : woff0[i - NP]) + (unsigned)(k0 * ldw * 4)));
    }
  };
  auto lstore = [&](int i, float* stage) {
    if (i < NP) st4(&stage[(sr + G::RPP * i) * LSR + sc], stg[i]);
    else st4(&stage[G::BREG + (cr + 8 * (i - NP)) * LSC + cc], stg[i]);
  };
  f32x16 acc[2][2];
#pragma unroll
  for (int i = 0; i < 2; ++i)
#pragma unroll
    for (int j = 0; j < 2; ++j) acc[i][j] = zero16();
  int s, k0;
  seg_of(0, s, k0);
#pragma unroll
  for (int i = 0; i < 2 * NP; ++i) gload_tile_piece(i, s, k0);
#pragma unroll
  for (int i = 0; i < 2 * NP; ++i) lstore(i, smem);
  seg_of(1, s, k0);
#pragma unroll
  for (int i = 0; i < 2 * NP; ++i) gload_tile_piece(i, s, k0);
  __syncthreads();
  int s2 = 0, k2 = 0;
  auto mv = [&](int i, float* nxt, int kt) {
    if (i == 0) seg_of(kt + 2, s2, k2);
    lstore(i, nxt);
    gload_tile_piece(i, s2, k2);
  };
  const int a_rd = (64 * wm + ln) * LSR + (BK / 2) * hf;
  const int b_rd = ((BK / 2) * hf) * LSC + 64 * wn + ln;
  __builtin_amdgcn_s_setprio(0);
  step_loop<BK, false, true>(acc, smem, nk, a_rd, 32 * LSR, b_rd, 32, mv);
  __builtin_amdgcn_s_setprio(AMK_DENSE_EDGE_PRIO);

  const float* cbase = p.c + m0 * p.ldc;
#pragma unroll
  for (int j = 0; j < 2; ++j) {
    const int n = n0 + 64 * wn + 32 * j + ln;
    const unsigned cn = n < p.N ? (unsigned)n * 4u : K_PAST;
    unsigned vo[4], va[4];
    lane_offsets(vo, hf, p.ldc, cn);
    if (EPI == EPI_SWIGLU_BWD) lane_offsets(va, hf, p.ldab, cn);
#pragma unroll
    for (int i = 0; i < 2; ++i) {
      if constexpr (EPI == EPI_SWIGLU_BWD) {
        const float* abbase = p.ab + m0 * p.ldab;
        float av[16], bv[16];
#pragma unroll
        for (int q = 0; q < 4; ++q) {
          const int rg0 = 64 * wm + 32 * i + 8 * q;
          const __amdgpu_buffer_rsrc_t ar = group_rsrc(abbase, p.ldab, rows, rg0, 0, p.H), br = group_rsrc(abbase, p.ldab, rows, rg0, p.H, p.H);
#pragma unroll
          for (int e = 0; e < 4; ++e) { av[4 * q + e] = bload1(ar, (int)va[e]); bv[4 * q + e] = bload1(br, (int)va[e]); }
        }
#pragma unroll
        for (int q = 0; q < 4; ++q) {
          const int rg0 = 64 * wm + 32 * i + 8 * q;
          const __amdgpu_buffer_rsrc_t dar = group_rsrc(cbase, p.ldc, rows, rg0, 0, p.H), dbr = group_rsrc(cbase, p.ldc, rows, rg0, p.H, p.H);
#pragma unroll
          for (int e = 0; e < 4; ++e) {
            const float g = acc[i][j][4 * q + e], a_ = av[4 * q + e], sg = sigmoidf_(a_);
            bstore1(g * bv[4 * q + e] * (sg * (1.f + a_ * (1.f - sg))), dar, (int)vo[e]);
            bstore1(g * (a_ * sg), dbr, (int)vo[e]);
          }
        }
      } else {
#pragma unroll
        for (int q = 0; q < 4; ++q) {
          const __amdgpu_buffer_rsrc_t cr_ = group_rsrc(cbase, p.ldc, rows, 64 * wm + 32 * i + 8 * q, 0, p.N);
#pragma unroll
          for (int e = 0; e < 4; ++e) bstore1(acc[i][j][4 * q + e], cr_, (int)vo[e]);
        }
      }
    }
  }
}

template <int BK, bool LNX>
__global__ AMK_DENSE_BOUNDS(BK) void gemm_tn_kernel(Params p) {
  using G = Geo<BK>;
  constexpr int NP = G::NP;
  __shared__ __attribute__((aligned(16))) float smem[2 * G::STAGE];
  const int tid = threadIdx.x, lane = tid & 63, wave = __builtin_amdgcn_readfirstlane(tid >> 6), ln = lane & 31, hf = lane >> 5;
  const int wm = wave >> 1, wn = wave & 1;
  stagger(p, (BK == 16 ? 3 : 2) * 256);
  __builtin_amdgcn_s_setprio(AMK_DENSE_EDGE_PRIO);
  const int u = xcd_remap(blockIdx.x, p.total);
  const int tile = u / p.nchunk, chunk = u - tile * p.nchunk;
  const int ntk = p.ntn;
  const int tn = tile / ntk, tk = tile - tn * ntk;
  int n0 = tn * 128;
  const int k0t = tk * 128;
  const bool seg = p.split > 0 && n0 >= p.split;
  const float* Yb = seg ? p.a2 : p.a;
  const int64_t ldy = seg ? p.lda2 : p.lda;
  const int nrows = p.split > 0 ? (seg ? p.N - p.split : p.split) : p.N;
  if (seg) n0 -= p.split;
  const int64_t mbeg = (int64_t)chunk * p.steps_per_chunk * BK;
  int64_t mend = mbeg + (int64_t)p.steps_per_chunk * BK;
  if (mend > p.M) mend = p.M;
  const int mrows = (int)(mend - mbeg);
  const int nk = (mrows + BK - 1) / BK;

  const int cr = tid >> 5, cc = (tid & 31) * 4;
  const __amdgpu_buffer_rsrc_t y_rsrc = mkrsrc(Yb + mbeg * ldy, ((int64_t)(mrows - 1) * ldy + nrows) * 4);
  const __amdgpu_buffer_rsrc_t x_rsrc = mkrsrc(p.w + mbeg * p.ldw, ((int64_t)(mrows - 1) * p.ldw + p.K) * 4);
  const __amdgpu_buffer_rsrc_t m_rsrc = mkrsrc(LNX ? p.ln_mean + mbeg : p.a, LNX ? (int64_t)mrows * 4 : 0);
  const __amdgpu_buffer_rsrc_t r_rsrc = mkrsrc(LNX ? p.ln_rstd + mbeg : p.a, LNX ? (int64_t)mrows * 4 : 0);
  const bool ycol_ok = n0 + cc < nrows, xcol_ok = k0t + cc < p.K;
  unsigned goff[2 * NP];
#pragma unroll
  for (int j = 0; j < NP; ++j) {
    goff[j] = ycol_ok ? (unsigned)(((int64_t)(cr + 8 * j) * ldy + n0 + cc) * 4) : ROW_PAST;
    goff[NP + j] = xcol_ok ? (unsigned)(((int64_t)(cr + 8 * j) * p.ldw + k0t + cc) * 4) : ROW_PAST;
  }
  const unsigned ystep = (unsigned)(BK * ldy * 4), xstep = (unsigned)(BK * p.ldw * 4);
  float4 gam = make_float4(0.f, 0.f, 0.f, 0.f), bet = gam;
  if (LNX && xcol_ok) { gam = ld4(p.ln_gamma + k0t + cc); bet = ld4(p.ln_beta + k0t + cc); }
  float4 stg[2 * NP];
  float mu[NP], rs[NP];
  float4 bsum = make_float4(0.f, 0.f, 0.f, 0.f);
  const bool do_bias = p.dbias != nullptr && tk == 0;
  auto gload = [&](int i, int kt) {
    const int t = kt < nk ? kt : nk - 1;
    if (i < NP) stg[i] = bload4(y_rsrc, (int)(goff[i] + (unsigned)t * ystep));
    else {
      stg[i] = bload4(x_rsrc, (int)(goff[i] + (unsigned)t * xstep));
      if (LNX) {
        mu[i - NP] = bload1(m_rsrc, (t * BK + cr + 8 * (i - NP)) * 4);
        rs[i - NP] = bload1(r_rsrc, (t * BK + cr + 8 * (i - NP)) * 4);
      }
    }
  };
  auto lstore = [&](int i, float* stage, bool count) {
    float4 v = stg[i];
    if (i < NP) {
      if (do_bias && count) { bsum.x += v.x; bsum.y += v.y; bsum.z += v.z; bsum.w += v.w; }
      st4(&stage[(cr + 8 * i) * LSC + cc], v);
    } else {
      if (LNX) {
        const float m_ = mu[i - NP], r_ = rs[i - NP];
        v.x = fmaf((v.x - m_) * r_, gam.x, bet.x); v.y = fmaf((v.y - m_) * r_, gam.y, bet.y);
        v.z = fmaf((v.z - m_) * r_, gam.z, bet.z); v.w = fmaf((v.w - m_) * r_, gam.w, bet.w);
      }
      st4(&stage[G::BREG + (cr + 8 * (i - NP)) * LSC + cc], v);
    }
  };
  f32x16 acc[2][2];
#pragma unroll
  for (int i = 0; i < 2; ++i)
#pragma unroll
    for (int j = 0; j < 2; ++j) acc[i][j] = zero16();
#pragma unroll
  for (int i = 0; i < 2 * NP; ++i) gload(i, 0);
#pragma unroll
  for (int i = 0; i < 2 * NP; ++i) lstore(i, smem, true);
#pragma unroll
  for (int i = 0; i < 2 * NP; ++i) gload(i, 1);
  __syncthreads();
  auto mv = [&](int i, float* nxt, int kt) {
    lstore(i, nxt, kt + 1 < nk);
    gload(i, kt + 2);
  };
  const int a_rd = ((BK / 2) * hf) * LSC + 64 * wm + ln;
  const int b_rd = ((BK / 2) * hf) * LSC + 64 * wn + ln;
  __builtin_amdgcn_s_setprio(0);
  step_loop<BK, true, true>(acc, smem, nk, a_rd, 32, b_rd, 32, mv);
  __builtin_amdgcn_s_setprio(AMK_DENSE_EDGE_PRIO);

  float* Cb;
  int64_t ldc;
  if (p.nchunk > 1) { Cb = p.ws + ((int64_t)chunk * p.N + (seg ? p.split : 0)) * p.K; ldc = p.K; }
  else { Cb = seg ? p.c2 : p.c; ldc = seg ? p.ldc2 : p.ldc; }
  const int orow = nrows - n0 < 128 ? nrows - n0 : 128;
  const float* cbase = Cb + (int64_t)n0 * ldc;
#pragma unroll
  for (int j = 0; j < 2; ++j) {
    const int kcol = k0t + 64 * wn + 32 * j + ln;
    const unsigned cn = kcol < p.K ? (unsigned)kcol * 4u : K_PAST;
    unsigned vo[4];
    lane_offsets(vo, hf, ldc, cn);
#pragma unroll
    for (int i = 0; i < 2; ++i) {
#pragma unroll
      for (int q = 0; q < 4; ++q) {
        const __amdgpu_buffer_rsrc_t cr_ = group_rsrc(cbase, ldc, orow, 64 * wm + 32 * i + 8 * q, 0, p.K);
#pragma unroll
        for (int e = 0; e < 4; ++e) bstore1(acc[i][j][4 * q + e], cr_, (int)vo[e]);
      }
    }
  }
  if (do_bias) {
    float* red = smem;
    st4(&red[cr * 128 + cc], bsum);
    __syncthreads();
    if (tid < 128) {
      float s = 0.f;
#pragma unroll
      for (int j = 0; j < 8; ++j) s += red[j * 128 + tid];
      const int n = n0 + tid;
      if (n < nrows) p.dbias[(int64_t)(p.nchunk > 1 ? chunk : 0) * p.N + (seg ? p.split : 0) + n] = s;
    }
  }
}

__global__ __launch_bounds__(256) void tn_reduce_kernel(Params p, float* dbias_out) {
  const int64_t total4 = (int64_t)p.N * p.K / 4;
  const int64_t slab = (int64_t)p.N * p.K;
  const int64_t i = (int64_t)blockIdx.x * 256 + threadIdx.x;
  if (i < total4) {
    const float* src = p.ws + 4 * i;
    float4 s = make_float4(0.f, 0.f, 0.f, 0.f);
    int c = 0;
    for (; c + 8 <= p.nchunk; c += 8) {
      float4 v[8];
#pragma unroll
      for (int j = 0; j < 8; ++j) v[j] = ld4(src + (c + j) * slab);
#pragma unroll
      for (int j = 0; j < 8; ++j) { s.x += v[j].x; s.y += v[j].y; s.z += v[j].z; s.w += v[j].w; }
    }
    for (; c < p.nchunk; ++c) {
      const float4 v = ld4(src + c * slab);
      s.x += v.x; s.y += v.y; s.z += v.z; s.w += v.w;
    }
    const int64_t e = 4 * i;
    const int64_t row = e / p.K;
    const int col = (int)(e - row * p.K);
    if (p.split > 0 && row >= p.split) st4(p.c2 + (row - p.split) * p.ldc2 + col, s);
    else st4(p.c + row * p.ldc + col, s);
  }
  if (dbias_out && blockIdx.x == gridDim.x - 1) {
    for (int n = threadIdx.x; n < p.N; n += 256) {
      float s = 0.f;
      for (int c = 0; c < p.nchunk; ++c) s += p.dbias[(int64_t)c * p.N + n];
      dbias_out[n] = s;
    }
  }
}

template <int NCH>
__global__ __launch_bounds__(256) void row_stats_kernel(const float* __restrict__ x, int64_t M, int D, float eps,
                                                        float* __restrict__ mean_out, float* __restrict__ rstd_out) {
  const int lane = threadIdx.x & 63, wave = threadIdx.x >> 6;
  const int nch = D >> 2;
  const float inv_d = 1.f / (float)D;
  for (int64_t row = (int64_t)blockIdx.x * 4 + wave; row < M; row += (int64_t)gridDim.x * 4) {
    float4 v[NCH];
    float s = 0.f;
#pragma unroll
    for (int j = 0; j < NCH; ++j) {
      const int c = lane + 64 * j;
      v[j] = c < nch ? ld4(x + row * D + 4 * c) : make_float4(0.f, 0.f, 0.f, 0.f);
      s += v[j].x + v[j].y + v[j].z + v[j].w;
    }
#pragma unroll
    for (int o = 32; o >= 1; o >>= 1) s += __shfl_xor(s, o, 64);
    const float mean = s * inv_d;
    float q = 0.f;
#pragma unroll
    for (int j = 0; j < NCH; ++j) {
      const int c = lane + 64 * j;
      if (c < nch) {
        const float a = v[j].x - mean, b = v[j].y - mean, cc = v[j].z - mean, d = v[j].w - mean;
        q += a * a + b * b + cc * cc + d * d;
      }
    }
#pragma unroll
    for (int o = 32; o >= 1; o >>= 1) q += __shfl_xor(q, o, 64);
    if (lane == 0) { mean_out[row] = mean; rstd_out[row] = rsqrtf(q * inv_d + eps); }
  }
}

}

using namespace amk_dense;

static bool a16(const void* p) { return (reinterpret_cast<uintptr_t>(p) & 15) == 0; }

static int dense_bk() {
  static int v = 0;
  if (v == 0) {
    const char* e = getenv("AMK_DENSE_BK");
    v = (e && atoi(e) == 32) ? 32 : ((e && atoi(e) == 16) ? 16 : AMK_DENSE_DEFAULT_BK);
  }
  return v;
}
static int wg_slots() {
  static int cus = 0;
  if (cus == 0) {
    int dev = 0;
    if (hipGetDevice(&dev) != hipSuccess || hipDeviceGetAttribute(&cus, hipDeviceAttributeMultiprocessorCount, dev) != hipSuccess || cus <= 0) cus = 256;
  }
  return (dense_bk() == 16 ? 3 : 2) * cus;
}

static int tn_chunks(const amk_gemm_desc* d, int* steps_per_chunk) {
  const int bk = dense_bk();
  const int tiles = ((d->n + 127) / 128) * ((d->k + 127) / 128);
  const int64_t steps = (d->m + bk - 1) / bk;
  const int64_t min_steps = 256 / bk;
  static int forced = -1;
  if (forced < 0) {
    const char* e = getenv("AMK_DENSE_TN_SLOTS");
    forced = e && atoi(e) > 0 ? atoi(e) : 0;
  }
  const int slots = forced ? forced : (tiles <= 16 ? wg_slots() / 2 : wg_slots());
  int64_t chunks = slots / tiles;
  if (chunks < 1) chunks = 1;
  if (chunks > steps / min_steps) chunks = steps / min_steps > 0 ? steps / min_steps : 1;
  int64_t spc = (steps + chunks - 1) / chunks;
  chunks = (steps + spc - 1) / spc;
  *steps_per_chunk = (int)spc;
  return (int)chunks;
}

extern "C" int64_t amk_gemm_f32_ws_bytes(const amk_gemm_desc* d) {
  if (!d || d->op != AMK_GEMM_TN) return 0;
  int spc;
  const int chunks = tn_chunks(d, &spc);
  if (chunks <= 1) return 0;
  return ((int64_t)chunks * d->n * d->k + (int64_t)chunks * d->n) * 4;
}

extern "C" int amk_row_stats(const float* x, int64_t M, int D, float eps, float* mean, float* rstd, void* stream) {
  AMK_CHECK_ARG(x && mean && rstd, "amk_row_stats: null pointer");
  AMK_CHECK_ARG(M > 0 && D > 0, "amk_row_stats: non-positive size");
  AMK_CHECK_SUPPORTED(D % 4 == 0 && D <= 4096 && a16(x), "amk_row_stats: D %% 4 == 0, D <= 4096 and a 16-byte aligned pointer required");
  const int64_t blocks = (M + 3) / 4;
  const dim3 grid((unsigned)(blocks < 16384 ? blocks : 16384));
  hipStream_t st = static_cast<hipStream_t>(stream);
  if (D <= 256) hipLaunchKernelGGL(row_stats_kernel<1>, grid, dim3(256), 0, st, x, M, D, eps, mean, rstd);
  else if (D <= 1024) hipLaunchKernelGGL(row_stats_kernel<4>, grid, dim3(256), 0, st, x, M, D, eps, mean, rstd);
  else hipLaunchKernelGGL(row_stats_kernel<16>, grid, dim3(256), 0, st, x, M, D, eps, mean, rstd);
  AMK_CHECK_LAUNCH("amk_row_stats");
  return AMK_OK;
}

extern "C" int amk_gemm_f32(const amk_gemm_desc* d, void* workspace, int64_t ws_bytes, void* stream) {
  AMK_CHECK_ARG(d, "amk_gemm_f32: null descriptor");
  const bool c_optional = d->op == AMK_GEMM_NT && d->epilogue == AMK_EPI_SWIGLU;
  AMK_CHECK_ARG(d->a && d->w && (d->c || c_optional), "amk_gemm_f32: null operand");
  AMK_CHECK_ARG(d->m > 0 && d->n > 0 && d->k > 0, "amk_gemm_f32: non-positive size");
  const bool two = d->split > 0;
  AMK_CHECK_SUPPORTED(d->k % 4 == 0 && d->lda % 4 == 0 && d->ldw % 4 == 0 && d->ldc % 4 == 0 && a16(d->a) && a16(d->w) && a16(d->c),
                      "amk_gemm_f32: K and leading dimensions must be multiples of 4, pointers 16-byte aligned");
  AMK_CHECK_SUPPORTED(d->m < (int64_t)1 << 31, "amk_gemm_f32: M too large");
  const int64_t lim = (int64_t)1 << 30;
  Params p = {};
  p.a = d->a; p.a2 = d->a2; p.w = d->w; p.w2 = d->w2; p.bias = d->bias; p.bias2 = d->bias2; p.resid = d->resid;
  p.c = d->c; p.c2 = d->c2;
  p.ln_mean = d->ln_mean; p.ln_rstd = d->ln_rstd; p.ln_gamma = d->ln_gamma; p.ln_beta = d->ln_beta;
  p.ab = d->ab; p.gate = d->gate;
  p.lda = d->lda; p.lda2 = d->lda2; p.ldw = d->ldw; p.ldw2 = d->ldw2; p.ldc = d->ldc; p.ldc2 = d->ldc2;
  p.ldr = d->ldr; p.ldab = d->ldab; p.ldg = d->ldg;
  p.M = d->m; p.N = d->n; p.K = d->k; p.split = d->split; p.H = d->n;
  {
    static int mode = -1, sleeps = 0;
    if (mode < 0) {
      const char* e = getenv("AMK_DENSE_STAGGER");
      mode = e ? atoi(e) : 0;
      const char* c = e ? strchr(e, ',') : nullptr;
      sleeps = c ? atoi(c + 1) : 2;
    }
    p.stagger_mode = mode; p.stagger_sleeps = sleeps;
  }
  const bool ln = d->ln_mean != nullptr;
  if (ln) AMK_CHECK_ARG(d->ln_rstd && d->ln_gamma && d->ln_beta, "amk_gemm_f32: LayerNorm operand needs mean, rstd, gamma and beta");
  if (two) {
    AMK_CHECK_ARG(d->split < (d->op == AMK_GEMM_NN ? d->k : d->n), "amk_gemm_f32: split outside the segmented axis");
    AMK_CHECK_SUPPORTED(d->split % 128 == 0 || d->op == AMK_GEMM_NN, "amk_gemm_f32: output split must be a multiple of 128");
    AMK_CHECK_SUPPORTED(d->op != AMK_GEMM_NN || d->split % 4 == 0, "amk_gemm_f32: contraction split must be a multiple of 4");
  }
  hipStream_t st = static_cast<hipStream_t>(stream);
  const int64_t mt = (d->m + 127) / 128;
  if (d->op == AMK_GEMM_NT) {
    const bool sw = d->epilogue == AMK_EPI_SWIGLU;
    if (two) AMK_CHECK_ARG(!sw && d->w2 && d->c2 && d->ldw2 % 4 == 0 && d->ldc2 % 4 == 0, "amk_gemm_f32: second column segment incomplete");
    AMK_CHECK_SUPPORTED(128 * d->lda * 4 < lim && (int64_t)(sw ? 2 : 1) * d->n * d->ldw * 4 < lim && 128 * d->ldc * 4 < lim,
                        "amk_gemm_f32: operand panel beyond 1 GiB");
    if (sw) AMK_CHECK_ARG(d->gate && d->ldg % 4 == 0, "amk_gemm_f32: SwiGLU epilogue needs the gate output");
    if (d->epilogue == AMK_EPI_RESID) AMK_CHECK_ARG(d->resid && !two && d->ldr % 4 == 0, "amk_gemm_f32: residual epilogue needs resid (one column segment)");
    p.ntn = sw ? (d->n + 63) / 64 : (two ? d->split / 128 + (d->n - d->split + 127) / 128 : (d->n + 127) / 128);
#ifdef AMK_DENSE_STAMPS
    p.ws = static_cast<float*>(workspace);
#endif
    const int64_t total = mt * p.ntn;
    AMK_CHECK_SUPPORTED(total < (int64_t)1 << 31, "amk_gemm_f32: grid too large");
    p.total = (int)total;
    const dim3 grid((unsigned)total), blk(256);
    const bool b16 = dense_bk() == 16;
    static int walk = -1;
    if (walk < 0) { const char* e = getenv("AMK_DENSE_WALK"); walk = (e && e[0] == '0') ? 0 : 1; }
    const bool use_walk = walk && !b16 && d->k > 96;
    const dim3 wgrid((unsigned)(total > wg_slots() ? wg_slots() : total));
#define AMK_NT(E, L) do { if (use_walk) hipLaunchKernelGGL((gemm_nt_dkernel<E, L>), wgrid, blk, 0, st, p); else if (b16) hipLaunchKernelGGL((gemm_nt_kernel<16, E, L>), grid, blk, 0, st, p); else hipLaunchKernelGGL((gemm_nt_kernel<32, E, L>), grid, blk, 0, st, p); } while (0)
    if (sw) { if (ln) AMK_NT(EPI_SWIGLU, true); else AMK_NT(EPI_SWIGLU, false); }
    else if (d->epilogue == AMK_EPI_RESID) { if (ln) AMK_NT(EPI_RESID, true); else AMK_NT(EPI_RESID, false); }
    else if (d->epilogue == AMK_EPI_BIAS) { if (ln) AMK_NT(EPI_BIAS, true); else AMK_NT(EPI_BIAS, false); }
    else AMK_CHECK_ARG(false, "amk_gemm_f32: epilogue %d is not an NT epilogue", d->epilogue);
#undef AMK_NT
    AMK_CHECK_LAUNCH("amk_gemm_f32(NT)");
    return AMK_OK;
  }
  if (d->op == AMK_GEMM_NN) {
    const bool swb = d->epilogue == AMK_EPI_SWIGLU_BWD;
    if (two) AMK_CHECK_ARG(d->a2 && d->w2 && d->lda2 % 4 == 0 && d->ldw2 % 4 == 0, "amk_gemm_f32: second contraction segment incomplete");
    AMK_CHECK_SUPPORTED(d->n % 4 == 0, "amk_gemm_f32(NN): N must be a multiple of 4");
    AMK_CHECK_SUPPORTED(128 * d->lda * 4 < lim && (int64_t)d->k * d->ldw * 4 < lim && 128 * d->ldc * 4 < lim &&
                        (!two || (128 * d->lda2 * 4 < lim && (int64_t)d->k * d->ldw2 * 4 < lim)),
                        "amk_gemm_f32: operand panel beyond 1 GiB");
    if (swb) AMK_CHECK_ARG(d->ab && d->ldab % 4 == 0 && 128 * d->ldab * 4 < lim, "amk_gemm_f32: SwiGLU backward epilogue needs (a | b)");
    else AMK_CHECK_ARG(d->epilogue == AMK_EPI_BIAS && !d->bias, "amk_gemm_f32(NN): epilogue must be AMK_EPI_BIAS without a bias, or AMK_EPI_SWIGLU_BWD");
    p.ntn = (d->n + 127) / 128;
    const int64_t total = mt * p.ntn;
    AMK_CHECK_SUPPORTED(total < (int64_t)1 << 31, "amk_gemm_f32: grid too large");
    p.total = (int)total;
    const dim3 grid((unsigned)total);
    const bool b16 = dense_bk() == 16;
    if (swb) { if (b16) hipLaunchKernelGGL((gemm_nn_kernel<16, EPI_SWIGLU_BWD>), grid, dim3(256), 0, st, p); else hipLaunchKernelGGL((gemm_nn_kernel<32, EPI_SWIGLU_BWD>), grid, dim3(256), 0, st, p); }
    else { if (b16) hipLaunchKernelGGL((gemm_nn_kernel<16, EPI_BIAS>), grid, dim3(256), 0, st, p); else hipLaunchKernelGGL((gemm_nn_kernel<32, EPI_BIAS>), grid, dim3(256), 0, st, p); }
    AMK_CHECK_LAUNCH("amk_gemm_f32(NN)");
    return AMK_OK;
  }
  AMK_CHECK_ARG(d->op == AMK_GEMM_TN, "amk_gemm_f32: unknown op %d", d->op);
  if (two) AMK_CHECK_ARG(d->a2 && d->c2 && d->lda2 % 4 == 0 && d->ldc2 % 4 == 0, "amk_gemm_f32: second row segment incomplete");
  AMK_CHECK_SUPPORTED(d->n % 4 == 0 && (!two || (d->n - d->split) % 4 == 0), "amk_gemm_f32(TN): N must be a multiple of 4");
  int spc;
  const int chunks = tn_chunks(d, &spc);
  AMK_CHECK_SUPPORTED((int64_t)spc * 32 * d->lda * 4 < lim && (int64_t)spc * 32 * d->ldw * 4 < lim && (!two || (int64_t)spc * 32 * d->lda2 * 4 < lim),
                      "amk_gemm_f32(TN): chunk panel beyond 1 GiB");
  AMK_CHECK_SUPPORTED((int64_t)d->n * d->k * 4 < lim, "amk_gemm_f32(TN): output beyond 1 GiB");
  if (chunks > 1) {
    AMK_CHECK_ARG(workspace && ws_bytes >= amk_gemm_f32_ws_bytes(d), "amk_gemm_f32(TN): workspace of amk_gemm_f32_ws_bytes() bytes required");
    AMK_CHECK_ARG(a16(workspace), "amk_gemm_f32(TN): workspace must be 16-byte aligned");
    p.ws = static_cast<float*>(workspace);
  }
  p.nchunk = chunks;
  p.steps_per_chunk = spc;
  p.ntn = (d->k + 127) / 128;
  float* dbias_out = d->dbias;
  p.dbias = d->dbias ? (chunks > 1 ? p.ws + (int64_t)chunks * d->n * d->k : d->dbias) : nullptr;
  const int64_t total = (int64_t)((d->n + 127) / 128) * p.ntn * chunks;
  if (two) AMK_CHECK_ARG(d->split % 128 == 0, "amk_gemm_f32(TN): split must be a multiple of 128");
  p.total = (int)total;
  {
    const dim3 grid((unsigned)total);
    const bool b16 = dense_bk() == 16;
    if (ln) { if (b16) hipLaunchKernelGGL((gemm_tn_kernel<16, true>), grid, dim3(256), 0, st, p); else hipLaunchKernelGGL((gemm_tn_kernel<32, true>), grid, dim3(256), 0, st, p); }
    else { if (b16) hipLaunchKernelGGL((gemm_tn_kernel<16, false>), grid, dim3(256), 0, st, p); else hipLaunchKernelGGL((gemm_tn_kernel<32, false>), grid, dim3(256), 0, st, p); }
  }
  AMK_CHECK_LAUNCH("amk_gemm_f32(TN)");
  if (chunks > 1) {
    const int64_t items = (int64_t)d->n * d->k / 4;
    const int64_t blocks = (items + 255) / 256;
    hipLaunchKernelGGL(tn_reduce_kernel, dim3((unsigned)blocks), dim3(256), 0, st, p, dbias_out);
    AMK_CHECK_LAUNCH("amk_gemm_f32(TN reduce)");
  }
  return AMK_OK;
}

extern "C" int amk_debug_dense_occupancy(int bk) {
  int n = -1;
  hipError_t e;
  if (bk == 16) e = hipOccupancyMaxActiveBlocksPerMultiprocessor(&n, gemm_nt_kernel<16, EPI_BIAS, false>, 256, 0);
  else e = hipOccupancyMaxActiveBlocksPerMultiprocessor(&n, gemm_nt_kernel<32, EPI_BIAS, false>, 256, 0);
  return e == hipSuccess ? n : -(int)e;
}
```

attention-models_amd/csrc/layernorm.hip:

```cpp
#include "amk_common.h"

namespace amk_ln {

__device__ __forceinline__ float4 ld4(const float* p) { return *reinterpret_cast<const float4*>(p); }
__device__ __forceinline__ void st4(float* p, float4 v) { *reinterpret_cast<float4*>(p) = v; }
__device__ __forceinline__ float wave_sum(float s) {
#pragma unroll
  for (int o = 32; o >= 1; o >>= 1) s += __shfl_xor(s, o, 64);
  return s;
}

constexpr int WAVES = 4;

template <int NCH, bool HAS_RES>
__global__ __launch_bounds__(64 * WAVES) void add_layernorm_fwd_kernel(
    const float* __restrict__ x, const float* __restrict__ res, const float* __restrict__ gamma,
    const float* __restrict__ beta, int64_t M, int D, float eps, float* __restrict__ h, float* __restrict__ y,
    float* __restrict__ mean_out, float* __restrict__ rstd_out) {
  const int lane = threadIdx.x & 63, wave = threadIdx.x >> 6;
  const int nch = D >> 2;
  float4 g[NCH], b[NCH];
#pragma unroll
  for (int j = 0; j < NCH; ++j) {
    const int c = lane + 64 * j;
    g[j] = c < nch ? ld4(gamma + 4 * c) : make_float4(0.f, 0.f, 0.f, 0.f);
    b[j] = c < nch ? ld4(beta + 4 * c) : make_float4(0.f, 0.f, 0.f, 0.f);
  }
  const float inv_d = 1.f / (float)D;
  for (int64_t row = (int64_t)blockIdx.x * WAVES + wave; row < M; row += (int64_t)gridDim.x * WAVES) {
    float4 v[NCH];
    float s = 0.f;
#pragma unroll
    for (int j = 0; j < NCH; ++j) {
      const int c = lane + 64 * j;
      v[j] = make_float4(0.f, 0.f, 0.f, 0.f);
      if (c < nch) {
        v[j] = ld4(x + row * D + 4 * c);
        if (HAS_RES) {
          const float4 r = ld4(res + row * D + 4 * c);
          v[j].x += r.x; v[j].y += r.y; v[j].z += r.z; v[j].w += r.w;
          st4(h + row * D + 4 * c, v[j]);
        }
        s += v[j].x + v[j].y + v[j].z + v[j].w;
      }
    }
    const float mean = wave_sum(s) * inv_d;
    float q = 0.f;
#pragma unroll
    for (int j = 0; j < NCH; ++j) {
      const int c = lane + 64 * j;
      if (c < nch) {
        v[j].x -= mean; v[j].y -= mean; v[j].z -= mean; v[j].w -= mean;
        q += v[j].x * v[j].x + v[j].y * v[j].y + v[j].z * v[j].z + v[j].w * v[j].w;
      }
    }
    const float rstd = rsqrtf(wave_sum(q) * inv_d + eps);
#pragma unroll
    for (int j = 0; j < NCH; ++j) {
      const int c = lane + 64 * j;
      if (c < nch)
        st4(y + row * D + 4 * c, make_float4(v[j].x * rstd * g[j].x + b[j].x, v[j].y * rstd * g[j].y + b[j].y,
                                             v[j].z * rstd * g[j].z + b[j].z, v[j].w * rstd * g[j].w + b[j].w));
    }
    if (lane == 0) { mean_out[row] = mean; rstd_out[row] = rstd; }
  }
}

template <int NCH, bool HAS_DH>
__global__ __launch_bounds__(64 * WAVES) void add_layernorm_bwd_kernel(
    const float* __restrict__ dy, const float* __restrict__ h, const float* __restrict__ dh_in,
    const float* __restrict__ gamma, const float* __restrict__ mean_in, const float* __restrict__ rstd_in,
    int64_t M, int D, float* __restrict__ dh, float* __restrict__ part) {
  extern __shared__ __attribute__((aligned(16))) float red[];
  const int lane = threadIdx.x & 63, wave = threadIdx.x >> 6;
  const int nch = D >> 2;
  float4 g[NCH], dg[NCH], db[NCH];
#pragma unroll
  for (int j = 0; j < NCH; ++j) {
    const int c = lane + 64 * j;
    g[j] = c < nch ? ld4(gamma + 4 * c) : make_float4(0.f, 0.f, 0.f, 0.f);
    dg[j] = make_float4(0.f, 0.f, 0.f, 0.f);
    db[j] = make_float4(0.f, 0.f, 0.f, 0.f);
  }
  const float inv_d = 1.f / (float)D;
  for (int64_t row = (int64_t)blockIdx.x * WAVES + wave; row < M; row += (int64_t)gridDim.x * WAVES) {
    const float mean = mean_in[row], rstd = rstd_in[row];
    float4 gy[NCH], xh[NCH];
    float s1 = 0.f, s2 = 0.f;
#pragma unroll
    for (int j = 0; j < NCH; ++j) {
      const int c = lane + 64 * j;
      gy[j] = make_float4(0.f, 0.f, 0.f, 0.f);
      xh[j] = make_float4(0.f, 0.f, 0.f, 0.f);
      if (c < nch) {
        const float4 d = ld4(dy + row * D + 4 * c);
        const float4 hv = ld4(h + row * D + 4 * c);
        xh[j] = make_float4((hv.x - mean) * rstd, (hv.y - mean) * rstd, (hv.z - mean) * rstd, (hv.w - mean) * rstd);
        gy[j] = make_float4(d.x * g[j].x, d.y * g[j].y, d.z * g[j].z, d.w * g[j].w);
        dg[j].x += d.x * xh[j].x; dg[j].y += d.y * xh[j].y; dg[j].z += d.z * xh[j].z; dg[j].w += d.w * xh[j].w;
        db[j].x += d.x; db[j].y += d.y; db[j].z += d.z; db[j].w += d.w;
        s1 += gy[j].x + gy[j].y + gy[j].z + gy[j].w;
        s2 += gy[j].x * xh[j].x + gy[j].y * xh[j].y + gy[j].z * xh[j].z + gy[j].w * xh[j].w;
      }
    }
    const float c1 = wave_sum(s1) * inv_d, c2 = wave_sum(s2) * inv_d;
#pragma unroll
    for (int j = 0; j < NCH; ++j) {
      const int c = lane + 64 * j;
      if (c < nch) {
        float4 o = make_float4(rstd * (gy[j].x - c1 - xh[j].x * c2), rstd * (gy[j].y - c1 - xh[j].y * c2),
                               rstd * (gy[j].z - c1 - xh[j].z * c2), rstd * (gy[j].w - c1 - xh[j].w * c2));
        if (HAS_DH) {
          const float4 a = ld4(dh_in + row * D + 4 * c);
          o.x += a.x; o.y += a.y; o.z += a.z; o.w += a.w;
        }
        st4(dh + row * D + 4 * c, o);
      }
    }
  }
#pragma unroll
  for (int pass = 0; pass < 2; ++pass) {
#pragma unroll
    for (int j = 0; j < NCH; ++j) {
      const int c = lane + 64 * j;
      if (c < nch) st4(&red[wave * D + 4 * c], pass == 0 ? dg[j] : db[j]);
    }
    __syncthreads();
    for (int i = threadIdx.x; i < D; i += 64 * WAVES) {
      float s = 0.f;
#pragma unroll
      for (int w = 0; w < WAVES; ++w) s += red[w * D + i];
      part[((int64_t)blockIdx.x * 2 + pass) * D + i] = s;
    }
    __syncthreads();
  }
}

template <int NCH>
__global__ __launch_bounds__(64 * WAVES) void colsum_kernel(const float* __restrict__ x, int64_t M, int N,
                                                            float* __restrict__ part) {
  extern __shared__ __attribute__((aligned(16))) float red[];
  const int lane = threadIdx.x & 63, wave = threadIdx.x >> 6;
  const int nch = N >> 2;
  float4 acc[NCH];
#pragma unroll
  for (int j = 0; j < NCH; ++j) acc[j] = make_float4(0.f, 0.f, 0.f, 0.f);
  for (int64_t row = (int64_t)blockIdx.x * WAVES + wave; row < M; row += (int64_t)gridDim.x * WAVES) {
#pragma unroll
    for (int j = 0; j < NCH; ++j) {
      const int c = lane + 64 * j;
      if (c < nch) {
        const float4 v = ld4(x + row * N + 4 * c);
        acc[j].x += v.x; acc[j].y += v.y; acc[j].z += v.z; acc[j].w += v.w;
      }
    }
  }
#pragma unroll
  for (int j = 0; j < NCH; ++j) {
    const int c = lane + 64 * j;
    if (c < nch) st4(&red[wave * N + 4 * c], acc[j]);
  }
  __syncthreads();
  for (int i = threadIdx.x; i < N; i += 64 * WAVES) {
    float s = 0.f;
#pragma unroll
    for (int w = 0; w < WAVES; ++w) s += red[w * N + i];
    part[(int64_t)blockIdx.x * N + i] = s;
  }
}

constexpr int MAX_D = 4096;
constexpr int MAX_PARTS = 2048;

}

using namespace amk_ln;

static bool a16(const void* p) { return (reinterpret_cast<uintptr_t>(p) & 15) == 0; }
static int parts_for(int64_t M) {
  const int64_t wg = (M + WAVES - 1) / WAVES;
  return (int)(wg < MAX_PARTS ? (wg > 0 ? wg : 1) : MAX_PARTS);
}
static unsigned fwd_grid(int64_t M) {
  const int64_t wg = (M + WAVES - 1) / WAVES;
  return (unsigned)(wg < 16384 ? (wg > 0 ? wg : 1) : 16384);
}

extern "C" int amk_rowsum_num_partials(int64_t M) { return M > 0 ? parts_for(M) : 0; }

#define AMK_LN_DISPATCH(D_, CALL)                     \
  do {                                                \
    if ((D_) <= 256) { CALL(1); }                     \
    else if ((D_) <= 512) { CALL(2); }                \
    else if ((D_) <= 1024) { CALL(4); }               \
    else if ((D_) <= 2048) { CALL(8); }               \
    else { CALL(16); }                                \
  } while (0)

extern "C" int amk_add_layernorm_fwd(const float* x, const float* res, const float* gamma, const float* beta,
                                     int64_t M, int D, float eps, float* h, float* y, float* mean, float* rstd,
                                     void* stream) {
  AMK_CHECK_ARG(x && gamma && beta && y && mean && rstd, "amk_add_layernorm_fwd: null pointer");
  AMK_CHECK_ARG((res == nullptr) == (h == nullptr), "amk_add_layernorm_fwd: res and h go together");
  AMK_CHECK_ARG(M > 0 && D > 0, "amk_add_layernorm_fwd: non-positive size");
  AMK_CHECK_SUPPORTED(D % 4 == 0 && D <= MAX_D, "amk_add_layernorm_fwd: width %d not supported (multiple of 4, <= %d)", D, MAX_D);
  AMK_CHECK_ARG(a16(x) && a16(res) && a16(gamma) && a16(beta) && a16(h) && a16(y), "amk_add_layernorm_fwd: pointers must be 16-byte aligned");
  hipStream_t st = static_cast<hipStream_t>(stream);
  const dim3 grid(fwd_grid(M)), block(64 * WAVES);
#define CALL(NCH)                                                                                                     \
  if (res) hipLaunchKernelGGL((add_layernorm_fwd_kernel<NCH, true>), grid, block, 0, st, x, res, gamma, beta, M, D, eps, h, y, mean, rstd); \
  else hipLaunchKernelGGL((add_layernorm_fwd_kernel<NCH, false>), grid, block, 0, st, x, res, gamma, beta, M, D, eps, h, y, mean, rstd)
  AMK_LN_DISPATCH(D, CALL);
#undef CALL
  AMK_CHECK_LAUNCH("amk_add_layernorm_fwd");
  return AMK_OK;
}

extern "C" int amk_add_layernorm_bwd(const float* dy, const float* h, const float* dh_in, const float* gamma,
                                     const float* mean, const float* rstd, int64_t M, int D, float* dh,
                                     float* dgb_part, void* stream) {
  AMK_CHECK_ARG(dy && h && gamma && mean && rstd && dh && dgb_part, "amk_add_layernorm_bwd: null pointer");
  AMK_CHECK_ARG(M > 0 && D > 0, "amk_add_layernorm_bwd: non-positive size");
  AMK_CHECK_SUPPORTED(D % 4 == 0 && D <= MAX_D, "amk_add_layernorm_bwd: width %d not supported (multiple of 4, <= %d)", D, MAX_D);
  AMK_CHECK_ARG(a16(dy) && a16(h) && a16(dh_in) && a16(gamma) && a16(dh) && a16(dgb_part), "amk_add_layernorm_bwd: pointers must be 16-byte aligned");
  hipStream_t st = static_cast<hipStream_t>(stream);
  const dim3 grid(parts_for(M)), block(64 * WAVES);
  const size_t lds = (size_t)WAVES * D * sizeof(float);
#define CALL(NCH)                                                                                                       \
  if (dh_in) hipLaunchKernelGGL((add_layernorm_bwd_kernel<NCH, true>), grid, block, lds, st, dy, h, dh_in, gamma, mean, rstd, M, D, dh, dgb_part); \
  else hipLaunchKernelGGL((add_layernorm_bwd_kernel<NCH, false>), grid, block, lds, st, dy, h, dh_in, gamma, mean, rstd, M, D, dh, dgb_part)
  AMK_LN_DISPATCH(D, CALL);
#undef CALL
  AMK_CHECK_LAUNCH("amk_add_layernorm_bwd");
  return AMK_OK;
}

extern "C" int amk_colsum(const float* x, int64_t M, int N, float* part, void* stream) {
  AMK_CHECK_ARG(x && part, "amk_colsum: null pointer");
  AMK_CHECK_ARG(M > 0 && N > 0, "amk_colsum: non-positive size");
  AMK_CHECK_SUPPORTED(N % 4 == 0 && N <= MAX_D, "amk_colsum: width %d not supported (multiple of 4, <= %d)", N, MAX_D);
  AMK_CHECK_ARG(a16(x) && a16(part), "amk_colsum: pointers must be 16-byte aligned");
  hipStream_t st = static_cast<hipStream_t>(stream);
  const dim3 grid(parts_for(M)), block(64 * WAVES);
  const size_t lds = (size_t)WAVES * N * sizeof(float);
#define CALL(NCH) hipLaunchKernelGGL(colsum_kernel<NCH>, grid, block, lds, st, x, M, N, part)
  AMK_LN_DISPATCH(N, CALL);
#undef CALL
  AMK_CHECK_LAUNCH("amk_colsum");
  return AMK_OK;
}
```

include/amk.h:

```cpp
#ifndef AMK_H_
#define AMK_H_

#include <stdint.h>

#ifdef __cplusplus
extern "C" {
#endif

#define AMK_VERSION 140

enum {
  AMK_OK = 0,
  AMK_EINVAL = -1,
  AMK_EUNSUPPORTED = -2,
  AMK_ELAUNCH = -3
};

int amk_version(void);
const char* amk_arch(void);
const char* amk_last_error(void);

int amk_attn_fwd(const float* q, const float* k, const float* v, float* o, float* stats,
                 const uint8_t* key_mask, const uint8_t* causal_mask,
                 int B, int H, int I, int J, int D,
                 int64_t q_sb, int64_t q_st, int64_t q_sh,
                 int64_t k_sb, int64_t k_st, int64_t k_sh,
                 int64_t v_sb, int64_t v_st, int64_t v_sh,
                 int64_t o_sb, int64_t o_st, int64_t o_sh,
                 float scale, void* stream);

int64_t amk_attn_scores_bytes(int B, int H, int I, int J);
int amk_attn_fwd_keep(const float* q, const float* k, const float* v, float* o, float* stats, float* scores,
                      const uint8_t* key_mask, const uint8_t* causal_mask,
                      int B, int H, int I, int J, int D,
                      int64_t q_sb, int64_t q_st, int64_t q_sh,
                      int64_t k_sb, int64_t k_st, int64_t k_sh,
                      int64_t v_sb, int64_t v_st, int64_t v_sh,
                      int64_t o_sb, int64_t o_st, int64_t o_sh,
                      float scale, void* stream);

int64_t amk_attn_fwd_x6_ws_bytes(int B, int H, int J);
int amk_attn_fwd_x6(const float* q, const float* k, const float* v, float* o, float* stats, void* ws,
                    const uint8_t* key_mask, const uint8_t* causal_mask,
                    int B, int H, int I, int J, int D,
                    int64_t q_sb, int64_t q_st, int64_t q_sh,
                    int64_t k_sb, int64_t k_st, int64_t k_sh,
                    int64_t v_sb, int64_t v_st, int64_t v_sh,
                    int64_t o_sb, int64_t o_st, int64_t o_sh,
                    float scale, void* stream);

#define AMK_ATTN_BWD_DELTA 1
#define AMK_ATTN_BWD_DKDV 2
#define AMK_ATTN_BWD_DQ 4
#define AMK_ATTN_BWD_FUSED 8
#define AMK_ATTN_BWD_ALL 7
#define AMK_ATTN_BWD_FAST 9
#define AMK_ATTN_BWD_KEYS128 16
#define AMK_ATTN_BWD_KEYS256 32
#define AMK_ATTN_BWD_DQ_REPRO 64
#define AMK_ATTN_BWD_FAST_REPRO 73
int64_t amk_attn_bwd_ws_floats(int B, int H, int I, int J, int stages);
int amk_attn_bwd(const float* q, const float* k, const float* v, const float* o,
                 const float* stats, const float* d_o,
                 float* dq, float* dk, float* dv, float* delta_ws,
                 const uint8_t* key_mask, const uint8_t* causal_mask,
                 int B, int H, int I, int J, int D,
                 int64_t q_sb, int64_t q_st, int64_t q_sh,
                 int64_t k_sb, int64_t k_st, int64_t k_sh,
                 int64_t v_sb, int64_t v_st, int64_t v_sh,
                 int64_t o_sb, int64_t o_st, int64_t o_sh,
                 int64_t do_sb, int64_t do_st, int64_t do_sh,
                 int64_t dq_sb, int64_t dq_st, int64_t dq_sh,
                 int64_t dk_sb, int64_t dk_st, int64_t dk_sh,
                 int64_t dv_sb, int64_t dv_st, int64_t dv_sh,
                 float scale, int stages, void* stream);
int amk_attn_bwd_kept(const float* scores, const float* q, const float* k, const float* v, const float* o,
                      const float* stats, const float* d_o,
                      float* dq, float* dk, float* dv, float* delta_ws,
                      const uint8_t* key_mask, const uint8_t* causal_mask,
                      int B, int H, int I, int J, int D,
                      int64_t q_sb, int64_t q_st, int64_t q_sh,
                      int64_t k_sb, int64_t k_st, int64_t k_sh,
                      int64_t v_sb, int64_t v_st, int64_t v_sh,
                      int64_t o_sb, int64_t o_st, int64_t o_sh,
                      int64_t do_sb, int64_t do_st, int64_t do_sh,
                      int64_t dq_sb, int64_t dq_st, int64_t dq_sh,
                      int64_t dk_sb, int64_t dk_st, int64_t dk_sh,
                      int64_t dv_sb, int64_t dv_st, int64_t dv_sh,
                      float scale, int stages, void* stream);

int64_t amk_vq_num_partials(int64_t N);
int amk_vq_padded_codes(int K, int nsplit);
int amk_vq_lookup_fwd(const float* z, const float* codebook, int64_t N, int K, int C, int nsplit,
                      float* en_ws, float* ee_ws, float* pmin_ws, int32_t* pidx_ws,
                      int64_t* idx, float* out, float* zq, float* zn, float* sqerr_partial,
                      void* stream);

int amk_vq_lookup_bwd(const float* z, const float* codebook, const float* zn, const float* zq,
                      const int64_t* idx, const float* g_out, const float* g_loss, float beta,
                      int64_t N, int K, int C, float* dz, float* dcodebook, void* stream);

int amk_vq_lookup_bwd_rows(const float* z, const float* codebook, const float* zn, const float* zq,
                           const int64_t* idx, const float* g_out, const float* g_loss, float beta,
                           int64_t N, int K, int C, float* dz, float* ge_rows, void* stream);

int amk_vq_gather(const int64_t* idx, const float* codebook, int64_t N, int K, int C,
                  float* out, int32_t* bad_count, void* stream);


int64_t amk_moe_route_ws_ints(int64_t U, int E, int k);
int amk_moe_route(const float* logits, int64_t U, int E, int k,
                  int64_t* ids, float* gate, int32_t* counts, int32_t* rank, int32_t* blockhist,
                  int32_t* offsets, int32_t* perm, void* stream);

int amk_grouped_gemm_nt(const float* A, int64_t lda, int a_div, const float* W, const float* bias,
                        const int32_t* offsets, const int32_t* perm, int64_t P, int E, int N, int Kd,
                        float* Y, void* stream);

int amk_grouped_gemm_nn(const float* A, int64_t lda, int a_div, const float* W, const float* scale,
                        const int32_t* offsets, const int32_t* perm, int64_t P, int E, int N, int Kd,
                        float* Y, void* stream);

int amk_grouped_gemm_nt_acc(const float* A, int64_t lda, int a_div, const float* W, const float* bias,
                            const int32_t* offsets, const int32_t* perm, int64_t P, int E, int N, int Kd,
                            float* Y, int y_div, void* stream);
int amk_grouped_gemm_nn_acc(const float* A, int64_t lda, int a_div, const float* W, const float* scale,
                            const int32_t* offsets, const int32_t* perm, int64_t P, int E, int N, int Kd,
                            float* Y, int y_div, void* stream);

int amk_grouped_gemm_wgrad(const float* G, int64_t ldg, int g_div, const float* X, int64_t ldx, int x_div,
                           const float* scale, const int32_t* offsets, const int32_t* perm,
                           int64_t P, int E, int N, int Kd, float* dW, float* dbias, void* stream);

int amk_moe_combine(const float* Y, const int64_t* ids, const float* scale, int64_t G, int outer, int k,
                    int N, float* out, void* stream);

int amk_moe_topk(const float* logits, int64_t U, int E, int k, int64_t* ids, float* gate, void* stream);

int amk_moe_route_distinct(const int64_t* ids, int64_t G, int fan, int E, uint64_t* mask,
                           int32_t* offsets, int32_t* perm, void* stream);

int amk_moe_combine_rows(const float* Y, const int64_t* ids, const float* scale, int64_t G, int outer, int k,
                         int N, int v_div, int E, float* out, void* stream);
int amk_moe_gate_grad_rows(const float* d_out, const float* Y, const int64_t* ids, const float* gate,
                           int64_t P, int k, int E, int N, int g_div, int v_div, float* dlogits, void* stream);

int amk_moe_expert_sums(const float* A, int64_t lda, int a_div, const int64_t* ids, const float* scale,
                        int64_t G, int fan, int E, int d, float* Z, void* stream);

int amk_moe_gate_grad(const float* d_out, const float* Y, const int64_t* ids, const float* gate,
                      int64_t P, int k, int E, int N, int g_div, float* dlogits, void* stream);

int amk_agent_num_chunks(int T);
int64_t amk_agent_ws_floats(int B, int H, int T, int P, int backward);
int amk_agent_num_chunks_dh(int T, int D);
int64_t amk_agent_ws_floats_dh(int B, int H, int T, int P, int D, int backward);

int amk_agent_attn_fwd(const float* q, const float* k, const float* v, const float* conv_w, const float* conv_b,
                       float* o, float* agents, float* vagent, float* stats1, float* ws,
                       int B, int H, int T, int D, int P,
                       int64_t q_sb, int64_t q_st, int64_t q_sh, int64_t k_sb, int64_t k_st, int64_t k_sh,
                       int64_t v_sb, int64_t v_st, int64_t v_sh, int64_t o_sb, int64_t o_st, int64_t o_sh,
                       float scale, void* stream);

int amk_agent_attn_bwd(const float* q, const float* k, const float* v, const float* conv_w, const float* d_o,
                       const float* agents, const float* vagent, const float* stats1,
                       float* dq, float* dk, float* dv, float* ws, float* dconvw_part, float* dconvb_part,
                       int B, int H, int T, int D, int P,
                       int64_t q_sb, int64_t q_st, int64_t q_sh, int64_t k_sb, int64_t k_st, int64_t k_sh,
                       int64_t v_sb, int64_t v_st, int64_t v_sh, int64_t do_sb, int64_t do_st, int64_t do_sh,
                       int64_t dq_sb, int64_t dq_st, int64_t dq_sh, int64_t dk_sb, int64_t dk_st, int64_t dk_sh,
                       int64_t dv_sb, int64_t dv_st, int64_t dv_sh, float scale, void* stream);

int amk_agent_conv_grad_reduce(const float* dconvw_part, const float* dconvb_part, int64_t rows, int D,
                               float* dconvw, float* dconvb, void* stream);

int amk_rowsum_num_partials(int64_t M);
int amk_add_layernorm_fwd(const float* x, const float* res, const float* gamma, const float* beta,
                          int64_t M, int D, float eps, float* h, float* y, float* mean, float* rstd, void* stream);
int amk_add_layernorm_bwd(const float* dy, const float* h, const float* dh_in, const float* gamma,
                          const float* mean, const float* rstd, int64_t M, int D, float* dh, float* dgb_part,
                          void* stream);
int amk_colsum(const float* x, int64_t M, int N, float* part, void* stream);

int amk_swiglu_fwd(const float* ab, int64_t M, int H, float* out, void* stream);
int amk_swiglu_bwd(const float* ab, const float* d_out, int64_t M, int H, float* d_ab, void* stream);

int amk_geglu_fwd(const float* ab, int64_t M, int H, float* out, void* stream);
int amk_geglu_bwd(const float* ab, const float* d_out, int64_t M, int H, float* d_ab, void* stream);

int amk_opt_num_partials(void);
int amk_sumsq_partials(const float* x, int64_t n, float* partials, void* stream);
int amk_adam_flat_step(float* param, float* grad, float* exp_avg, float* exp_avg_sq, int64_t n,
                       const int32_t* seg_param, const float* param_tab,
                       const float* partials, int n_partials,
                       float max_norm, float lr, float beta1, float beta2, float eps, float weight_decay,
                       int decoupled, float* norm_out, void* stream);
int amk_adam_flat_step_shadow(float* param, float* grad, float* exp_avg, float* exp_avg_sq, int64_t n,
                              const int32_t* seg_param, const float* param_tab,
                              const float* partials, int n_partials,
                              float max_norm, float lr, float beta1, float beta2, float eps, float weight_decay,
                              int decoupled, float* norm_out, void* param_bf16, void* stream);

int amk_sample_step(const float* logits, const float* null_logits, float cfg_scale,
                    const float* gumbel, uint64_t seed, uint64_t offset, float tau,
                    int64_t R, int V, int keep, const uint8_t* mask, float unmasked_score,
                    int64_t* ids, float* scores, void* stream);

int64_t amk_gemm_x6_planes_bytes(int N, int K);
int amk_gemm_x6_split(const float* W, int64_t ldw, int N, int K, void* planes, void* stream);
int amk_gemm_x6_nt(const float* A, int64_t lda, const void* w_planes, const float* bias,
                   float* C, int64_t ldc, int M, int N, int K, void* stream);

enum { AMK_GEMM_NT = 0, AMK_GEMM_NN = 1, AMK_GEMM_TN = 2 };
enum { AMK_EPI_BIAS = 0, AMK_EPI_RESID = 1, AMK_EPI_SWIGLU = 2, AMK_EPI_SWIGLU_BWD = 3 };
typedef struct amk_gemm_desc {
  int32_t op, epilogue;
  int64_t m;
  int32_t n, k, split, reserved;
  const float *a, *a2, *w, *w2;
  float *c, *c2;
  int64_t lda, lda2, ldw, ldw2, ldc, ldc2;
  const float *bias, *bias2, *resid;
  int64_t ldr;
  const float *ln_mean, *ln_rstd, *ln_gamma, *ln_beta;
  const float* ab;
  int64_t ldab;
  float* gate;
  int64_t ldg;
  float* dbias;
} amk_gemm_desc;
int64_t amk_gemm_f32_ws_bytes(const amk_gemm_desc* d);
int amk_gemm_f32(const amk_gemm_desc* d, void* workspace, int64_t ws_bytes, void* stream);
int amk_row_stats(const float* x, int64_t M, int D, float eps, float* mean, float* rstd, void* stream);

int amk_attn_bf16_fwd(const void* q, const void* k, const void* v, void* o, float* stats,
                      const uint8_t* key_mask, const uint8_t* causal_mask,
                      int B, int H, int I, int J, int D,
                      int64_t q_sb, int64_t q_st, int64_t q_sh, int64_t k_sb, int64_t k_st, int64_t k_sh,
                      int64_t v_sb, int64_t v_st, int64_t v_sh, int64_t o_sb, int64_t o_st, int64_t o_sh,
                      float scale, void* stream);
int64_t amk_attn_bf16_bwd_ws_floats(int B, int H, int I, int J);
int amk_attn_bf16_bwd(const void* q, const void* k, const void* v, const void* o, const float* stats, const void* d_o,
                      void* dq, void* dk, void* dv, float* ws,
                      const uint8_t* key_mask, const uint8_t* causal_mask,
                      int B, int H, int I, int J, int D,
                      int64_t q_sb, int64_t q_st, int64_t q_sh, int64_t k_sb, int64_t k_st, int64_t k_sh,
                      int64_t v_sb, int64_t v_st, int64_t v_sh, int64_t o_sb, int64_t o_st, int64_t o_sh,
                      int64_t do_sb, int64_t do_st, int64_t do_sh, int64_t dq_sb, int64_t dq_st, int64_t dq_sh,
                      int64_t dk_sb, int64_t dk_st, int64_t dk_sh, int64_t dv_sb, int64_t dv_st, int64_t dv_sh,
                      float scale, void* stream);

int amk_swiglu_bf16_fwd(const void* ab, int64_t M, int H, void* out, void* stream);
int amk_swiglu_bf16_bwd(const void* ab, const void* d_out, int64_t M, int H, void* d_ab, void* stream);
int amk_add_layernorm_mixed_fwd(const void* x, int x_is_bf16, const float* res, const float* gamma, const float* beta,
                                int64_t M, int D, float eps, float* h, void* y_bf16, float* mean, float* rstd, void* stream);
int amk_add_layernorm_mixed_bwd(const void* dy, int dy_is_bf16, const float* h, const float* dh_in, const float* gamma,
                                const float* mean, const float* rstd, int64_t M, int D, float* dh, void* dh_bf16,
                                float* dgb_part, void* stream);

int64_t amk_gemm_tn_bf16_ws_bytes(int64_t M, int N, int K);
int amk_gemm_tn_bf16(const void* y, int64_t ldy, const void* x, int64_t ldx, float* c, int64_t ldc, float* dbias,
                     int64_t M, int N, int K, void* workspace, int64_t ws_bytes, void* stream);

int amk_gemm_bf16(int op, int epi, const void* a, int64_t lda, const void* w, int64_t ldw, const float* bias,
                  void* c, int64_t ldc, void* g, int64_t ldg, int64_t M, int N, int K, void* stream);

int amk_gemm_bf16_swiglu_bwd(const void* dy, int64_t lddy, const void* w3, int64_t ldw, const void* ab, int64_t ldab,
                             void* dab, int64_t lddab, int64_t M, int H, int K, void* stream);

int64_t amk_bnact_ws_floats(int N, int C, int64_t HW);
int amk_bnact_fwd(const float* x, const float* gamma, const float* beta, int N, int C, int64_t HW, float eps,
                  float momentum, float slope, float* z, float* mean, float* rstd, float* running_mean,
                  float* running_var, float* ws, void* stream);
int amk_bnact_bwd(const float* gz, const float* x, const float* gamma, const float* beta, const float* mean,
                  const float* rstd, int N, int C, int64_t HW, float slope, float* gx, float* sums, float* dgamma,
                  float* dbeta, float* ws, void* stream);
int amk_bnact_bwd_bwd(const float* ggx, const float* gg_gamma, const float* gg_beta, const float* gz, const float* x,
                      const float* gamma, const float* beta, const float* mean, const float* rstd, const float* sums,
                      int N, int C, int64_t HW, float slope, float* g_gz, float* g_x, float* g_gamma, float* ws,
                      void* stream);

#ifdef __cplusplus
}
#endif
#endif
```

Baseline: 306.9 images/s.

## Fold split-K TN reduction and LayerNorm param-grad reduction into last-arriving blocks

```diff
diff --git a/attention-models_amd/amk/dense.py b/attention-models_amd/amk/dense.py
--- a/attention-models_amd/amk/dense.py
+++ b/attention-models_amd/amk/dense.py
@@ -3,7 +3,8 @@
 import torch
 
 from . import lib as _lib
-from .lib import EPI_BIAS, EPI_RESID, EPI_SWIGLU, EPI_SWIGLU_BWD, GEMM_NN, GEMM_NT, GEMM_TN, GemmDesc
+from .lib import (EPI_BIAS, EPI_RESID, EPI_SWIGLU, EPI_SWIGLU_BWD, GEMM_NN, GEMM_NT, GEMM_TN, GEMM_TN_COUNT_BYTES,
+                  GemmDesc)
 
 
 def _p(t):
@@ -140,6 +141,30 @@
             or t.data_ptr() % 16):
         raise RuntimeError(f"{what}: an fp32 contiguous 16-byte aligned HIP tensor of shape {tuple(shape)} is required")
     return t
+
+
+_tn_ws = {}
+_tn_ws_outgrown = []
+
+
+def _zeroed_counts(nfloats, device):
+    ws = torch.empty((nfloats,), device=device, dtype=torch.float32)
+    ws[:GEMM_TN_COUNT_BYTES // 4].zero_()
+    return ws
+
+
+def tn_workspace(nbytes, device):
+    key = torch.device(device).index
+    ws = _tn_ws.get(key)
+    if ws is not None and ws.numel() * 4 >= nbytes:
+        return ws
+    if torch.cuda.is_current_stream_capturing():
+        return _zeroed_counts(nbytes // 4, device)
+    if ws is not None:
+        _tn_ws_outgrown.append(ws)
+    grown = max(nbytes, ws.numel() * 6 if ws is not None else 0)
+    ws = _tn_ws[key] = _zeroed_counts((grown + 3) // 4, device)
+    return ws
 
 
 def gemm_tn(y, x, *, y2=None, ln=None, want_bias=False, out=None, out2=None, bias_out=None):
@@ -169,7 +194,7 @@
     keep = _set_ln(d, ln, M, K)
     L = _lib.load()
     nbytes = L.amk_gemm_f32_ws_bytes(ctypes.byref(d))
-    ws = torch.empty((nbytes // 4,), device=y.device, dtype=torch.float32) if nbytes else None
+    ws = tn_workspace(nbytes, y.device) if nbytes else None
     _run(d, ws)
     return dw, dw2, db
 
diff --git a/attention-models_amd/amk/lib.py b/attention-models_amd/amk/lib.py
--- a/attention-models_amd/amk/lib.py
+++ b/attention-models_amd/amk/lib.py
@@ -27,6 +27,8 @@
 
 
 GEMM_NT, GEMM_NN, GEMM_TN = 0, 1, 2
+GEMM_TN_COUNT_BYTES = 16384
+LN_COUNT_WORDS = 128
 EPI_BIAS, EPI_RESID, EPI_SWIGLU, EPI_SWIGLU_BWD = 0, 1, 2, 3
 
 SIGNATURES = {
@@ -57,6 +59,8 @@
     "amk_rowsum_num_partials": (_I, [_L]),
     "amk_add_layernorm_fwd": (_I, [_P, _P, _P, _P, _L, _I, _F, _P, _P, _P, _P, _P]),
     "amk_add_layernorm_bwd": (_I, [_P, _P, _P, _P, _P, _P, _L, _I, _P, _P, _P]),
+    "amk_add_layernorm_bwd_params_part_floats": (_L, [_L, _I]),
+    "amk_add_layernorm_bwd_params": (_I, [_P, _P, _P, _P, _P, _P, _L, _I, _P, _P, _P, _P, _P, _P]),
     "amk_colsum": (_I, [_P, _L, _I, _P, _P]),
     "amk_swiglu_fwd": (_I, [_P, _L, _I, _P, _P]),
     "amk_swiglu_bwd": (_I, [_P, _P, _L, _I, _P, _P]),
diff --git a/attention-models_amd/amk/ops.py b/attention-models_amd/amk/ops.py
--- a/attention-models_amd/amk/ops.py
+++ b/attention-models_amd/amk/ops.py
@@ -940,14 +940,48 @@
     return _claim(p)
 
 
+_ln_counts = {}
+
+
+def _ln_arrival_counts(device):
+    key = device.index
+    c = _ln_counts.get(key)
+    if c is None:
+        c = torch.zeros((_lib.LN_COUNT_WORDS,), device=device, dtype=torch.int32)
+        if torch.cuda.is_current_stream_capturing():
+            return c
+        _ln_counts[key] = c
+    return c
+
+
+def _grad_target(p, like):
+    r, v = _claim_late(p)
+    if v is not None and v.is_contiguous() and v.dtype == torch.float32 and v.numel() == like.numel():
+        return r, v
+    return None, torch.empty((like.numel(),), device=like.device, dtype=torch.float32)
+
+
 def _ln_backward(dy, h, dh_in, weight, mean, rstd, params=None):
     M, D = h.shape
     L = _lib.load()
     dh = torch.empty_like(h)
-    part = torch.empty((L.amk_rowsum_num_partials(M), 2, D), device=h.device, dtype=torch.float32)
-    _lib.check(L.amk_add_layernorm_bwd(_ptr(dy), _ptr(h), _ptr(dh_in), _ptr(weight), _ptr(mean), _ptr(rstd),
-                                       M, D, _ptr(dh), _ptr(part), _stream()), "amk_add_layernorm_bwd")
-    dw, db = _ln_param_grads(part, params)
+    if os.environ.get("AMK_LN_TWO_LAUNCH", "0") == "1":
+        part = torch.empty((L.amk_rowsum_num_partials(M), 2, D), device=h.device, dtype=torch.float32)
+        _lib.check(L.amk_add_layernorm_bwd(_ptr(dy), _ptr(h), _ptr(dh_in), _ptr(weight), _ptr(mean), _ptr(rstd),
+                                           M, D, _ptr(dh), _ptr(part), _stream()), "amk_add_layernorm_bwd")
+        return (dh, *_ln_param_grads(part, params))
+    part = torch.empty((L.amk_add_layernorm_bwd_params_part_floats(M, D),), device=h.device, dtype=torch.float32)
+    pw, pb = params if params is not None else (None, None)
+    (wr, dw), (br, db) = _grad_target(pw, weight), _grad_target(pb, weight)
+    _lib.check(L.amk_add_layernorm_bwd_params(_ptr(dy), _ptr(h), _ptr(dh_in), _ptr(weight), _ptr(mean), _ptr(rstd),
+                                              M, D, _ptr(dh), _ptr(part), _ptr(dw), _ptr(db),
+                                              _ptr(_ln_arrival_counts(h.device)), _stream()), "amk_add_layernorm_bwd_params")
+    if wr is not None:
+        wr.wrote(pw)
+        dw = None
+    if br is not None:
+        br.wrote(pb)
+        db = None
     return dh, dw, db
 
 
diff --git a/attention-models_amd/csrc/amk_common.h b/attention-models_amd/csrc/amk_common.h
--- a/attention-models_amd/csrc/amk_common.h
+++ b/attention-models_amd/csrc/amk_common.h
@@ -53,6 +53,32 @@
   return base + (bid >> 3);
 }
 
+template <bool RELEASE = true>
+__device__ __forceinline__ bool amk_last_arrival(unsigned* count, unsigned expected, unsigned* flag) {
+  asm volatile("s_waitcnt vmcnt(0)" ::: "memory");
+  __syncthreads();
+  if (threadIdx.x == 0) {
+    if (RELEASE) {
+      __builtin_amdgcn_fence(__ATOMIC_RELEASE, "agent");
+      asm volatile("s_waitcnt vmcnt(0)" ::: "memory");
+    }
+    const unsigned old = __hip_atomic_fetch_add(count, 1u, __ATOMIC_RELAXED, __HIP_MEMORY_SCOPE_AGENT);
+    const bool last = old + 1u == expected;
+    if (last) {
+      __hip_atomic_store(count, 0u, __ATOMIC_RELAXED, __HIP_MEMORY_SCOPE_AGENT);
+      __builtin_amdgcn_fence(__ATOMIC_ACQUIRE, "agent");
+      asm volatile("s_waitcnt vmcnt(0)" ::: "memory");
+    }
+    *flag = last ? 1u : 0u;
+  }
+  __syncthreads();
+  return *flag != 0u;
+}
+
+__device__ __forceinline__ void amk_store_through(float* p, float v) {
+  __hip_atomic_store(p, v, __ATOMIC_RELAXED, __HIP_MEMORY_SCOPE_AGENT);
+}
+
 __device__ __forceinline__ float wave_xor32_max(float x) {
   return fmaxf(x, __shfl_xor(x, 32, 64));
 }
diff --git a/attention-models_amd/csrc/gemm_f32.hip b/attention-models_amd/csrc/gemm_f32.hip
--- a/attention-models_amd/csrc/gemm_f32.hip
+++ b/attention-models_amd/csrc/gemm_f32.hip
@@ -46,6 +46,9 @@
 __device__ __forceinline__ __amdgpu_buffer_rsrc_t mkrsrc(const void* base, int64_t bytes) {
   return __builtin_amdgcn_make_buffer_rsrc((void*)base, 0, (int)(bytes < 0 ? 0 : (bytes > 0x3FFFFFFF ? 0x3FFFFFFF : bytes)), 0x00020000);
 }
+__device__ __forceinline__ __amdgpu_buffer_rsrc_t mkrsrc32(const void* base, int bytes) {
+  return __builtin_amdgcn_make_buffer_rsrc((void*)base, 0, bytes < 0 ? 0 : bytes, 0x00020000);
+}
 __device__ __forceinline__ float sigmoidf_(float x) { return 1.f / (1.f + expf(-x)); }
 
 __device__ __forceinline__ void lds_barrier() {
@@ -64,6 +67,8 @@
   float* gate;
   float* dbias;
   float* ws;
+  unsigned* cnt;
+  float* dbias_out;
   int64_t lda, lda2, ldw, ldw2, ldc, ldc2, ldr, ldab, ldg;
   int64_t M;
   int N, K, split, H;
@@ -766,10 +771,6 @@
   const int nk = (mrows + BK - 1) / BK;
 
   const int cr = tid >> 5, cc = (tid & 31) * 4;
-  const __amdgpu_buffer_rsrc_t y_rsrc = mkrsrc(Yb + mbeg * ldy, ((int64_t)(mrows - 1) * ldy + nrows) * 4);
-  const __amdgpu_buffer_rsrc_t x_rsrc = mkrsrc(p.w + mbeg * p.ldw, ((int64_t)(mrows - 1) * p.ldw + p.K) * 4);
-  const __amdgpu_buffer_rsrc_t m_rsrc = mkrsrc(LNX ? p.ln_mean + mbeg : p.a, LNX ? (int64_t)mrows * 4 : 0);
-  const __amdgpu_buffer_rsrc_t r_rsrc = mkrsrc(LNX ? p.ln_rstd + mbeg : p.a, LNX ? (int64_t)mrows * 4 : 0);
   const bool ycol_ok = n0 + cc < nrows, xcol_ok = k0t + cc < p.K;
   unsigned goff[2 * NP];
 #pragma unroll
@@ -777,36 +778,25 @@
     goff[j] = ycol_ok ? (unsigned)(((int64_t)(cr + 8 * j) * ldy + n0 + cc) * 4) : ROW_PAST;
     goff[NP + j] = xcol_ok ? (unsigned)(((int64_t)(cr + 8 * j) * p.ldw + k0t + cc) * 4) : ROW_PAST;
   }
-  const unsigned ystep = (unsigned)(BK * ldy * 4), xstep = (unsigned)(BK * p.ldw * 4);
   float4 gam = make_float4(0.f, 0.f, 0.f, 0.f), bet = gam;
   if (LNX && xcol_ok) { gam = ld4(p.ln_gamma + k0t + cc); bet = ld4(p.ln_beta + k0t + cc); }
   float4 stg[2 * NP];
   float mu[NP], rs[NP];
   float4 bsum = make_float4(0.f, 0.f, 0.f, 0.f);
   const bool do_bias = p.dbias != nullptr && tk == 0;
+  const float* ybase = Yb + mbeg * ldy;
+  const float* xbase = p.w + mbeg * p.ldw;
+  const int ldy_ = (int)ldy, ldx_ = (int)p.ldw;
   auto gload = [&](int i, int kt) {
-    const int t = kt < nk ? kt : nk - 1;
-    if (i < NP) stg[i] = bload4(y_rsrc, (int)(goff[i] + (unsigned)t * ystep));
-    else {
-      stg[i] = bload4(x_rsrc, (int)(goff[i] + (unsigned)t * xstep));
+    const int r0 = kt * BK, left = mrows - r0;
+    if (i < NP) {
+      stg[i] = bload4(mkrsrc32(ybase + (int64_t)r0 * ldy, ((left - 1) * ldy_ + nrows) * 4), (int)goff[i]);
+    } else {
+      stg[i] = bload4(mkrsrc32(xbase + (int64_t)r0 * p.ldw, ((left - 1) * ldx_ + p.K) * 4), (int)goff[i]);
       if (LNX) {
-        mu[i - NP] = bload1(m_rsrc, (t * BK + cr + 8 * (i - NP)) * 4);
-        rs[i - NP] = bload1(r_rsrc, (t * BK + cr + 8 * (i - NP)) * 4);
-      }
-    }
-  };
-  auto lstore = [&](int i, float* stage, bool count) {
-    float4 v = stg[i];
-    if (i < NP) {
-      if (do_bias && count) { bsum.x += v.x; bsum.y += v.y; bsum.z += v.z; bsum.w += v.w; }
-      st4(&stage[(cr + 8 * i) * LSC + cc], v);
-    } else {
-      if (LNX) {
-        const float m_ = mu[i - NP], r_ = rs[i - NP];
-        v.x = fmaf((v.x - m_) * r_, gam.x, bet.x); v.y = fmaf((v.y - m_) * r_, gam.y, bet.y);
-        v.z = fmaf((v.z - m_) * r_, gam.z, bet.z); v.w = fmaf((v.w - m_) * r_, gam.w, bet.w);
-      }
-      st4(&stage[G::BREG + (cr + 8 * (i - NP)) * LSC + cc], v);
+        mu[i - NP] = bload1(mkrsrc32(p.ln_mean + mbeg + r0, left * 4), (cr + 8 * (i - NP)) * 4);
+        rs[i - NP] = bload1(mkrsrc32(p.ln_rstd + mbeg + r0, left * 4), (cr + 8 * (i - NP)) * 4);
+      }
     }
   };
   f32x16 acc[2][2];
@@ -814,21 +804,40 @@
   for (int i = 0; i < 2; ++i)
 #pragma unroll
     for (int j = 0; j < 2; ++j) acc[i][j] = zero16();
-#pragma unroll
-  for (int i = 0; i < 2 * NP; ++i) gload(i, 0);
-#pragma unroll
-  for (int i = 0; i < 2 * NP; ++i) lstore(i, smem, true);
-#pragma unroll
-  for (int i = 0; i < 2 * NP; ++i) gload(i, 1);
-  __syncthreads();
-  auto mv = [&](int i, float* nxt, int kt) {
-    lstore(i, nxt, kt + 1 < nk);
-    gload(i, kt + 2);
-  };
   const int a_rd = ((BK / 2) * hf) * LSC + 64 * wm + ln;
   const int b_rd = ((BK / 2) * hf) * LSC + 64 * wn + ln;
-  __builtin_amdgcn_s_setprio(0);
-  step_loop<BK, true, true>(acc, smem, nk, a_rd, 32, b_rd, 32, mv);
+  auto body = [&](auto bias_tag) {
+    constexpr bool BIAS = decltype(bias_tag)::value;
+    auto lstore = [&](int i, float* stage) {
+      float4 v = stg[i];
+      if (i < NP) {
+        if constexpr (BIAS) { bsum.x += v.x; bsum.y += v.y; bsum.z += v.z; bsum.w += v.w; }
+        st4(&stage[(cr + 8 * i) * LSC + cc], v);
+      } else {
+        if (LNX) {
+          const float m_ = mu[i - NP], r_ = rs[i - NP];
+          v.x = fmaf((v.x - m_) * r_, gam.x, bet.x); v.y = fmaf((v.y - m_) * r_, gam.y, bet.y);
+          v.z = fmaf((v.z - m_) * r_, gam.z, bet.z); v.w = fmaf((v.w - m_) * r_, gam.w, bet.w);
+        }
+        st4(&stage[G::BREG + (cr + 8 * (i - NP)) * LSC + cc], v);
+      }
+    };
+#pragma unroll
+    for (int i = 0; i < 2 * NP; ++i) gload(i, 0);
+#pragma unroll
+    for (int i = 0; i < 2 * NP; ++i) lstore(i, smem);
+#pragma unroll
+    for (int i = 0; i < 2 * NP; ++i) gload(i, 1);
+    __syncthreads();
+    auto mv = [&](int i, float* nxt, int kt) {
+      lstore(i, nxt);
+      gload(i, kt + 2);
+    };
+    __builtin_amdgcn_s_setprio(0);
+    step_loop<BK, true, true>(acc, smem, nk, a_rd, 32, b_rd, 32, mv);
+  };
+  if (do_bias) body(std::true_type{});
+  else body(std::false_type{});
   __builtin_amdgcn_s_setprio(AMK_DENSE_EDGE_PRIO);
 
   float* Cb;
@@ -863,6 +872,56 @@
       for (int j = 0; j < 8; ++j) s += red[j * 128 + tid];
       const int n = n0 + tid;
       if (n < nrows) p.dbias[(int64_t)(p.nchunk > 1 ? chunk : 0) * p.N + (seg ? p.split : 0) + n] = s;
+    }
+  }
+  if (p.nchunk > 1 && p.cnt != nullptr) {
+    if (!amk_last_arrival(p.cnt + tile, (unsigned)p.nchunk, reinterpret_cast<unsigned*>(smem))) return;
+    const int64_t slab = (int64_t)p.N * p.K;
+    const float* src0 = p.ws + (int64_t)((seg ? p.split : 0) + n0) * p.K + k0t;
+    const int64_t ldo = seg ? p.ldc2 : p.ldc;
+    float* dst0 = (seg ? p.c2 : p.c) + (int64_t)n0 * ldo + k0t;
+    constexpr int PC = 2;
+    for (int it = 0; it < 16; it += PC) {
+      float4 s[PC];
+      const float* src[PC];
+      bool ok[PC];
+      int r_[PC], c_[PC];
+#pragma unroll
+      for (int u_ = 0; u_ < PC; ++u_) {
+        const int idx = tid + 256 * (it + u_);
+        r_[u_] = idx >> 5; c_[u_] = (idx & 31) * 4;
+        ok[u_] = r_[u_] < orow && k0t + c_[u_] < p.K;
+        src[u_] = src0 + (int64_t)r_[u_] * p.K + c_[u_];
+        s[u_] = make_float4(0.f, 0.f, 0.f, 0.f);
+      }
+      int c = 0;
+      for (; c + 8 <= p.nchunk; c += 8) {
+        float4 v[PC][8];
+#pragma unroll
+        for (int u_ = 0; u_ < PC; ++u_)
+#pragma unroll
+          for (int j = 0; j < 8; ++j) v[u_][j] = ok[u_] ? ld4(src[u_] + (c + j) * slab) : make_float4(0.f, 0.f, 0.f, 0.f);
+#pragma unroll
+        for (int u_ = 0; u_ < PC; ++u_)
+#pragma unroll
+          for (int j = 0; j < 8; ++j) { s[u_].x += v[u_][j].x; s[u_].y += v[u_][j].y; s[u_].z += v[u_][j].z; s[u_].w += v[u_][j].w; }
+      }
+      for (; c < p.nchunk; ++c) {
+        float4 v[PC];
+#pragma unroll
+        for (int u_ = 0; u_ < PC; ++u_) v[u_] = ok[u_] ? ld4(src[u_] + c * slab) : make_float4(0.f, 0.f, 0.f, 0.f);
+#pragma unroll
+        for (int u_ = 0; u_ < PC; ++u_) { s[u_].x += v[u_].x; s[u_].y += v[u_].y; s[u_].z += v[u_].z; s[u_].w += v[u_].w; }
+      }
+#pragma unroll
+      for (int u_ = 0; u_ < PC; ++u_)
+        if (ok[u_]) st4(dst0 + (int64_t)r_[u_] * ldo + c_[u_], s[u_]);
+    }
+    if (do_bias && p.dbias_out != nullptr && tid < 128 && n0 + tid < nrows) {
+      const int n = (seg ? p.split : 0) + n0 + tid;
+      float s = 0.f;
+      for (int c = 0; c < p.nchunk; ++c) s += p.dbias[(int64_t)c * p.N + n];
+      p.dbias_out[n] = s;
     }
   }
 }
@@ -962,11 +1021,8 @@
   const int tiles = ((d->n + 127) / 128) * ((d->k + 127) / 128);
   const int64_t steps = (d->m + bk - 1) / bk;
   const int64_t min_steps = 256 / bk;
-  static int forced = -1;
-  if (forced < 0) {
-    const char* e = getenv("AMK_DENSE_TN_SLOTS");
-    forced = e && atoi(e) > 0 ? atoi(e) : 0;
-  }
+  const char* e = getenv("AMK_DENSE_TN_SLOTS");
+  const int forced = e && atoi(e) > 0 ? atoi(e) : 0;
   const int slots = forced ? forced : (tiles <= 16 ? wg_slots() / 2 : wg_slots());
   int64_t chunks = slots / tiles;
   if (chunks < 1) chunks = 1;
@@ -977,12 +1033,18 @@
   return (int)chunks;
 }
 
+static bool tn_finish_in_kernel(int64_t tiles, int chunks) {
+  const char* e = getenv("AMK_TN_TWO_LAUNCH");
+  if (e && (e[0] == '0' || e[0] == '1')) return e[0] == '0';
+  return tiles >= 32 && chunks <= 16;
+}
+
 extern "C" int64_t amk_gemm_f32_ws_bytes(const amk_gemm_desc* d) {
   if (!d || d->op != AMK_GEMM_TN) return 0;
   int spc;
   const int chunks = tn_chunks(d, &spc);
   if (chunks <= 1) return 0;
-  return ((int64_t)chunks * d->n * d->k + (int64_t)chunks * d->n) * 4;
+  return AMK_GEMM_TN_COUNT_BYTES + ((int64_t)chunks * d->n * d->k + (int64_t)chunks * d->n) * 4;
 }
 
 extern "C" int amk_row_stats(const float* x, int64_t M, int D, float eps, float* mean, float* rstd, void* stream) {
@@ -1096,12 +1158,15 @@
   if (chunks > 1) {
     AMK_CHECK_ARG(workspace && ws_bytes >= amk_gemm_f32_ws_bytes(d), "amk_gemm_f32(TN): workspace of amk_gemm_f32_ws_bytes() bytes required");
     AMK_CHECK_ARG(a16(workspace), "amk_gemm_f32(TN): workspace must be 16-byte aligned");
-    p.ws = static_cast<float*>(workspace);
+    p.ws = reinterpret_cast<float*>(static_cast<char*>(workspace) + AMK_GEMM_TN_COUNT_BYTES);
+    const int64_t tiles = (int64_t)((d->n + 127) / 128) * ((d->k + 127) / 128);
+    if (tn_finish_in_kernel(tiles, chunks) && tiles * 4 <= AMK_GEMM_TN_COUNT_BYTES) p.cnt = static_cast<unsigned*>(workspace);
   }
   p.nchunk = chunks;
   p.steps_per_chunk = spc;
   p.ntn = (d->k + 127) / 128;
   float* dbias_out = d->dbias;
+  p.dbias_out = d->dbias;
   p.dbias = d->dbias ? (chunks > 1 ? p.ws + (int64_t)chunks * d->n * d->k : d->dbias) : nullptr;
   const int64_t total = (int64_t)((d->n + 127) / 128) * p.ntn * chunks;
   if (two) AMK_CHECK_ARG(d->split % 128 == 0, "amk_gemm_f32(TN): split must be a multiple of 128");
@@ -1113,7 +1178,7 @@
     else { if (b16) hipLaunchKernelGGL((gemm_tn_kernel<16, false>), grid, dim3(256), 0, st, p); else hipLaunchKernelGGL((gemm_tn_kernel<32, false>), grid, dim3(256), 0, st, p); }
   }
   AMK_CHECK_LAUNCH("amk_gemm_f32(TN)");
-  if (chunks > 1) {
+  if (chunks > 1 && p.cnt == nullptr) {
     const int64_t items = (int64_t)d->n * d->k / 4;
     const int64_t blocks = (items + 255) / 256;
     hipLaunchKernelGGL(tn_reduce_kernel, dim3((unsigned)blocks), dim3(256), 0, st, p, dbias_out);
diff --git a/attention-models_amd/csrc/layernorm.hip b/attention-models_amd/csrc/layernorm.hip
--- a/attention-models_amd/csrc/layernorm.hip
+++ b/attention-models_amd/csrc/layernorm.hip
@@ -11,6 +11,7 @@
 }
 
 constexpr int WAVES = 4;
+constexpr int FOLD = AMK_LN_FOLD_GROUP;
 
 template <int NCH, bool HAS_RES>
 __global__ __launch_bounds__(64 * WAVES) void add_layernorm_fwd_kernel(
@@ -70,7 +71,8 @@
 __global__ __launch_bounds__(64 * WAVES) void add_layernorm_bwd_kernel(
     const float* __restrict__ dy, const float* __restrict__ h, const float* __restrict__ dh_in,
     const float* __restrict__ gamma, const float* __restrict__ mean_in, const float* __restrict__ rstd_in,
-    int64_t M, int D, float* __restrict__ dh, float* __restrict__ part) {
+    int64_t M, int D, float* __restrict__ dh, float* part, float* __restrict__ dgamma, float* __restrict__ dbeta,
+    unsigned* counts) {
   extern __shared__ __attribute__((aligned(16))) float red[];
   const int lane = threadIdx.x & 63, wave = threadIdx.x >> 6;
   const int nch = D >> 2;
@@ -130,10 +132,39 @@
       float s = 0.f;
 #pragma unroll
       for (int w = 0; w < WAVES; ++w) s += red[w * D + i];
-      part[((int64_t)blockIdx.x * 2 + pass) * D + i] = s;
+      if (counts != nullptr) amk_store_through(&part[((int64_t)blockIdx.x * 2 + pass) * D + i], s);
+      else part[((int64_t)blockIdx.x * 2 + pass) * D + i] = s;
     }
     __syncthreads();
   }
+  if (counts == nullptr) return;
+  const int parts = gridDim.x, ngroups = (parts + FOLD - 1) / FOLD, grp = blockIdx.x / FOLD;
+  const int W = 2 * D;
+  float* gsum = part + (int64_t)parts * W;
+  auto fold = [&](const float* src, int rows, float* dst) {
+    for (int e = threadIdx.x; e < W; e += 64 * WAVES) {
+      float s = 0.f;
+      int r = 0;
+      for (; r + 8 <= rows; r += 8) {
+        float v[8];
+#pragma unroll
+        for (int j = 0; j < 8; ++j) v[j] = src[(int64_t)(r + j) * W + e];
+#pragma unroll
+        for (int j = 0; j < 8; ++j) s += v[j];
+      }
+      for (; r < rows; ++r) s += src[(int64_t)r * W + e];
+      if (dst) amk_store_through(&dst[e], s);
+      else if (e < D) dgamma[e] = s;
+      else dbeta[e - D] = s;
+    }
+  };
+  unsigned* arrived = reinterpret_cast<unsigned*>(red);
+  const int g0 = grp * FOLD, gn = parts - g0 < FOLD ? parts - g0 : FOLD;
+  if (!amk_last_arrival<false>(counts + 1 + grp, (unsigned)gn, arrived)) return;
+  fold(part + (int64_t)g0 * W, gn, ngroups == 1 ? nullptr : gsum + (int64_t)grp * W);
+  if (ngroups == 1) return;
+  if (!amk_last_arrival<false>(counts, (unsigned)ngroups, arrived)) return;
+  fold(gsum, ngroups, nullptr);
 }
 
 template <int NCH>
@@ -171,6 +202,7 @@
 
 constexpr int MAX_D = 4096;
 constexpr int MAX_PARTS = 2048;
+static_assert(1 + (MAX_PARTS + FOLD - 1) / FOLD <= AMK_LN_COUNT_WORDS, "one count word per group and one for the groups");
 
 }
 
@@ -216,9 +248,9 @@
   return AMK_OK;
 }
 
-extern "C" int amk_add_layernorm_bwd(const float* dy, const float* h, const float* dh_in, const float* gamma,
-                                     const float* mean, const float* rstd, int64_t M, int D, float* dh,
-                                     float* dgb_part, void* stream) {
+static int ln_bwd(const float* dy, const float* h, const float* dh_in, const float* gamma, const float* mean,
+                  const float* rstd, int64_t M, int D, float* dh, float* dgb_part, float* dgamma, float* dbeta,
+                  unsigned* counts, void* stream) {
   AMK_CHECK_ARG(dy && h && gamma && mean && rstd && dh && dgb_part, "amk_add_layernorm_bwd: null pointer");
   AMK_CHECK_ARG(M > 0 && D > 0, "amk_add_layernorm_bwd: non-positive size");
   AMK_CHECK_SUPPORTED(D % 4 == 0 && D <= MAX_D, "amk_add_layernorm_bwd: width %d not supported (multiple of 4, <= %d)", D, MAX_D);
@@ -227,12 +259,32 @@
   const dim3 grid(parts_for(M)), block(64 * WAVES);
   const size_t lds = (size_t)WAVES * D * sizeof(float);
 #define CALL(NCH)                                                                                                       \
-  if (dh_in) hipLaunchKernelGGL((add_layernorm_bwd_kernel<NCH, true>), grid, block, lds, st, dy, h, dh_in, gamma, mean, rstd, M, D, dh, dgb_part); \
-  else hipLaunchKernelGGL((add_layernorm_bwd_kernel<NCH, false>), grid, block, lds, st, dy, h, dh_in, gamma, mean, rstd, M, D, dh, dgb_part)
+  if (dh_in) hipLaunchKernelGGL((add_layernorm_bwd_kernel<NCH, true>), grid, block, lds, st, dy, h, dh_in, gamma, mean, rstd, M, D, dh, dgb_part, dgamma, dbeta, counts); \
+  else hipLaunchKernelGGL((add_layernorm_bwd_kernel<NCH, false>), grid, block, lds, st, dy, h, dh_in, gamma, mean, rstd, M, D, dh, dgb_part, dgamma, dbeta, counts)
   AMK_LN_DISPATCH(D, CALL);
 #undef CALL
   AMK_CHECK_LAUNCH("amk_add_layernorm_bwd");
   return AMK_OK;
+}
+
+extern "C" int amk_add_layernorm_bwd(const float* dy, const float* h, const float* dh_in, const float* gamma,
+                                     const float* mean, const float* rstd, int64_t M, int D, float* dh,
+                                     float* dgb_part, void* stream) {
+  return ln_bwd(dy, h, dh_in, gamma, mean, rstd, M, D, dh, dgb_part, nullptr, nullptr, nullptr, stream);
+}
+
+extern "C" int64_t amk_add_layernorm_bwd_params_part_floats(int64_t M, int D) {
+  if (M <= 0 || D <= 0) return 0;
+  const int parts = parts_for(M);
+  return (int64_t)(parts + (parts + FOLD - 1) / FOLD) * 2 * D;
+}
+
+extern "C" int amk_add_layernorm_bwd_params(const float* dy, const float* h, const float* dh_in, const float* gamma,
+                                            const float* mean, const float* rstd, int64_t M, int D, float* dh,
+                                            float* dgb_part, float* dgamma, float* dbeta, uint32_t* counts,
+                                            void* stream) {
+  AMK_CHECK_ARG(dgamma && dbeta && counts, "amk_add_layernorm_bwd_params: null pointer");
+  return ln_bwd(dy, h, dh_in, gamma, mean, rstd, M, D, dh, dgb_part, dgamma, dbeta, counts, stream);
 }
 
 extern "C" int amk_colsum(const float* x, int64_t M, int N, float* part, void* stream) {
diff --git a/include/amk.h b/include/amk.h
--- a/include/amk.h
+++ b/include/amk.h
@@ -181,6 +181,12 @@
 int amk_add_layernorm_bwd(const float* dy, const float* h, const float* dh_in, const float* gamma,
                           const float* mean, const float* rstd, int64_t M, int D, float* dh, float* dgb_part,
                           void* stream);
+#define AMK_LN_FOLD_GROUP 32
+#define AMK_LN_COUNT_WORDS 128
+int64_t amk_add_layernorm_bwd_params_part_floats(int64_t M, int D);
+int amk_add_layernorm_bwd_params(const float* dy, const float* h, const float* dh_in, const float* gamma,
+                                 const float* mean, const float* rstd, int64_t M, int D, float* dh, float* dgb_part,
+                                 float* dgamma, float* dbeta, uint32_t* counts, void* stream);
 int amk_colsum(const float* x, int64_t M, int N, float* part, void* stream);
 
 int amk_swiglu_fwd(const float* ab, int64_t M, int H, float* out, void* stream);
@@ -212,6 +218,7 @@
 int amk_gemm_x6_nt(const float* A, int64_t lda, const void* w_planes, const float* bias,
                    float* C, int64_t ldc, int M, int N, int K, void* stream);
 
+#define AMK_GEMM_TN_COUNT_BYTES 16384
 enum { AMK_GEMM_NT = 0, AMK_GEMM_NN = 1, AMK_GEMM_TN = 2 };
 enum { AMK_EPI_BIAS = 0, AMK_EPI_RESID = 1, AMK_EPI_SWIGLU = 2, AMK_EPI_SWIGLU_BWD = 3 };
 typedef struct amk_gemm_desc {
```

After: 307.0 images/s (median of 3 runs). Within noise of the previous version (+0.1%).
